# kocurvik/mdrp

Measured on AMD Instinct MI355X. Metric: image-pairs/sec (2000 corrs, 10k RANSAC iters), higher is better.
Workload: dtype f64

## Files before the change

mdrp_amd/csrc/mdrp_capi.hip:

```cpp
#include "../../include/mdrp.h"
#include "mdrp_kernels.h"
#include "mdrp_classic.h"
#include "mdrp_frontend.h"
#ifdef MDRP_SPLIT_TU
#define MDRP_INST extern
#include "mdrp_instances.h"
namespace mdrp {
MDRP_INSTANCES_FINAL_64
MDRP_INSTANCES_FINAL_256
MDRP_INSTANCES_CLASSIC
}
#endif

#include <algorithm>
#include <cmath>
#include <cstdio>
#include <cstdlib>
#include <cstddef>
#include <cstring>
#include <functional>
#include <map>
#include <memory>
#include <mutex>
#include <string>
#include <vector>

using namespace mdrp;

static_assert(sizeof(mdrp_model) == sizeof(Model), "model layout");
static_assert(sizeof(mdrp_camera) == sizeof(CamDev), "camera layout");
static_assert(sizeof(mdrp_result) == sizeof(ResultDev), "result layout");

namespace {

thread_local std::string g_err;

#define HIPCHK(expr)                                                                                       \
    do {                                                                                                   \
        hipError_t e_ = (expr);                                                                            \
        if (e_ != hipSuccess) {                                                                            \
            char buf_[512];                                                                                \
            snprintf(buf_, sizeof buf_, "%s failed: %s (%s:%d)", #expr, hipGetErrorString(e_), __FILE__, __LINE__); \
            g_err = buf_;                                                                                  \
            return MDRP_ERR_HIP;                                                                           \
        }                                                                                                  \
    } while (0)

struct DevBuf {
    void *p = nullptr;
    size_t cap = 0;
    DevBuf() = default;
    DevBuf(const DevBuf &) = delete;
    DevBuf &operator=(const DevBuf &) = delete;
    ~DevBuf() { release(); }
    int ensure(size_t bytes) {
        if (bytes <= cap) return MDRP_OK;
        if (p) { (void)hipFree(p); p = nullptr; cap = 0; }
        size_t want = bytes + bytes / 8 + 256;
        hipError_t e = hipMalloc(&p, want);
        if (e != hipSuccess) { g_err = std::string("hipMalloc failed: ") + hipGetErrorString(e); p = nullptr; return MDRP_ERR_HIP; }
        cap = want;
        return MDRP_OK;
    }
    void release() { if (p) (void)hipFree(p); p = nullptr; cap = 0; }
    template <typename T> T *as() const { return reinterpret_cast<T *>(p); }
};

template <typename T, auto Destroy> struct Owned {
    T v = nullptr;
    Owned() = default;
    Owned(Owned &&o) noexcept : v(o.v) { o.v = nullptr; }
    Owned(const Owned &) = delete;
    Owned &operator=(const Owned &) = delete;
    ~Owned() { reset(); }
    void reset() { if (v) (void)Destroy(v); v = nullptr; }
    operator T() const { return v; }
    T operator->() const { return v; }
};
using Stream = Owned<hipStream_t, hipStreamDestroy>;
using Event = Owned<hipEvent_t, hipEventDestroy>;
template <typename T> using Pinned = Owned<T *, hipHostFree>;

struct Progress {
    int32_t n_active, pad_;
    unsigned long long max_needed;
    unsigned long long evals;
    unsigned long long evals_mfma;
    unsigned long long evals_sweep;
    unsigned long long evals_bound;
    int32_t wish_sum, wish_pairs;
};
struct Counters {
    int32_t unused_[2];
    Progress progress;
    int32_t lo_head[16];
    int32_t xcd_head[8 * LO_XCD_STRIDE];
};
static_assert(offsetof(Counters, progress) == 2 * sizeof(int32_t) && offsetof(Counters, lo_head) == 16 * sizeof(int32_t) &&
              offsetof(Counters, xcd_head) == 32 * sizeof(int32_t) && sizeof(Counters) == 640, "counter block layout");
static_assert(offsetof(Progress, evals_mfma) == offsetof(Progress, evals) + sizeof(unsigned long long), "k_count adds to stats[0] and stats[1]");
static_assert(offsetof(Progress, wish_pairs) == offsetof(Progress, wish_sum) + sizeof(int32_t), "RunParams::inl_stat is [2]");
constexpr size_t LM_STATS_BYTES = 6 * sizeof(unsigned long long);

struct DeviceGuard {
    int prev = -1;
    bool ok = true;
    explicit DeviceGuard(int device) {
        if (hipGetDevice(&prev) != hipSuccess) prev = -1;
        if (prev != device) ok = hipSetDevice(device) == hipSuccess;
    }
    ~DeviceGuard() {
        int cur = -1;
        if (prev >= 0 && hipGetDevice(&cur) == hipSuccess && cur != prev) (void)hipSetDevice(prev);
    }
};

}

struct mdrp_handle {
    std::mutex mu;
    int device = 0;
    hipStream_t stream = nullptr;
    Stream own_stream;
    Stream aux_stream;
    Stream aux_stream2;
    Stream copy_stream;
    Event ev_copied, ev_prepped, ev_solved6;
    DevBuf fuse;
    static constexpr int NC_MAX = 8;
    Event ev_lo, ev_tables, ev_sampled[2], ev_solved[NC_MAX], ev_scanned[NC_MAX];
    int num_cu = 256;
    DevBuf pts, dep, st;
    DevBuf params;
    Pinned<unsigned char> params_host;
    size_t params_host_cap = 0;
    DevBuf models, slot_score, slot_inl, triggers, work_pair, counters, results, mask, plan;
    DevBuf samples[2], tags[2], model_count[2];
    DevBuf tags_sorted[2];
    DevBuf tags_v, surv_count;
    DevBuf cand_stat;
    DevBuf und_count;
    DevBuf rfrag;
    DevBuf cplan;
    DevBuf surv2_count;
    DevBuf lo_mask;
    DevBuf red5;
    DevBuf lm_stats;
    Pinned<unsigned long long> lm_stats_host;
    int64_t fuse_gate_timeouts = 0, fuse_wait_timeouts = 0;
    int64_t first_chunk = 0;
    double seen_wish[3] = {-1.0, -1.0, -1.0};
    Pinned<int32_t> wish_host; Event ev_wish;
    int wish_kind = -1;
    bool fuse_disabled = false;
    int fuse_retry_in = 0;
    int fuse_backoff = 64;
    DevBuf ckpt, ck_list, bresults, bmask;
    int last_budgets = 0;
    DevBuf in_x1, in_x2, in_d1, in_d2;
    DevBuf fe_x1, fe_x2, fe_d1, fe_d2, fe_slot, fe_n;
    Pinned<int32_t> fe_n_host;
    size_t fe_n_host_cap = 0;
    DevBuf unit_a, unit_b, unit_c, unit_d, unit_e, unit_f;
    Pinned<Progress> progress_host;
    std::vector<std::pair<Event, Event>> ev_pool;
    std::vector<int> ev_what;
    size_t ev_used = 0;
    double sweep_ms = 0.0, count_ms = 0.0;
    double kind_ms[6] = {0, 0, 0, 0, 0, 0};
    int64_t kind_launches[6] = {0, 0, 0, 0, 0, 0};
    int64_t lm_cost_evals = 0, lm_accum_evals = 0, fin_cost_evals = 0, fin_accum_evals = 0;
    int64_t count_launches = 0;
    int64_t sweep_launches = 0, sweep_evals = 0, mfma_evals = 0, fp64_evals = 0, bound_evals = 0;
    int last_batch = 0;
};

namespace {

#define MDRP_LM_DISPATCH_T(KERNEL, T, kind, shift, grid, smem, stream, ...)                                          \
    do {                                                                                                             \
        if ((kind) == 0 && (shift)) hipLaunchKernelGGL((KERNEL<0, true, T>), grid, dim3(T), smem, stream, __VA_ARGS__);  \
        else if ((kind) == 0) hipLaunchKernelGGL((KERNEL<0, false, T>), grid, dim3(T), smem, stream, __VA_ARGS__);       \
        else if ((kind) == 1) hipLaunchKernelGGL((KERNEL<1, false, T>), grid, dim3(T), smem, stream, __VA_ARGS__);       \
        else hipLaunchKernelGGL((KERNEL<2, false, T>), grid, dim3(T), smem, stream, __VA_ARGS__);                        \
    } while (0)
#define MDRP_LM_DISPATCH(KERNEL, threads, kind, shift, grid, smem, stream, ...)                                      \
    do {                                                                                                             \
        if ((threads) == 64) MDRP_LM_DISPATCH_T(KERNEL, 64, kind, shift, grid, smem, stream, __VA_ARGS__);           \
        else MDRP_LM_DISPATCH_T(KERNEL, 256, kind, shift, grid, smem, stream, __VA_ARGS__);                          \
    } while (0)

#define MDRP_FINAL_DISPATCH_L(T, FL, kind, shift, grid, smem, stream, ...)                                                  \
    do {                                                                                                                   \
        if ((kind) == 0 && (shift)) hipLaunchKernelGGL((k_final<0, true, T, FL>), grid, dim3(T), smem, stream, __VA_ARGS__);  \
        else if ((kind) == 0) hipLaunchKernelGGL((k_final<0, false, T, FL>), grid, dim3(T), smem, stream, __VA_ARGS__);       \
        else if ((kind) == 1) hipLaunchKernelGGL((k_final<1, false, T, FL>), grid, dim3(T), smem, stream, __VA_ARGS__);       \
        else hipLaunchKernelGGL((k_final<2, false, T, FL>), grid, dim3(T), smem, stream, __VA_ARGS__);                        \
    } while (0)
#define MDRP_FINAL_DISPATCH_T(T, floss, kind, shift, grid, smem, stream, ...)                                               \
    do {                                                                                                                   \
        switch (floss) {                                                                                                   \
        case 1: MDRP_FINAL_DISPATCH_L(T, 1, kind, shift, grid, smem, stream, __VA_ARGS__); break;                          \
        case 2: MDRP_FINAL_DISPATCH_L(T, 2, kind, shift, grid, smem, stream, __VA_ARGS__); break;                          \
        case 3: MDRP_FINAL_DISPATCH_L(T, 3, kind, shift, grid, smem, stream, __VA_ARGS__); break;                          \
        case 4: MDRP_FINAL_DISPATCH_L(T, 4, kind, shift, grid, smem, stream, __VA_ARGS__); break;                          \
        case 5: MDRP_FINAL_DISPATCH_L(T, 5, kind, shift, grid, smem, stream, __VA_ARGS__); break;                          \
        default: MDRP_FINAL_DISPATCH_L(T, 0, kind, shift, grid, smem, stream, __VA_ARGS__); break;  \
        }                                                                                                                  \
    } while (0)
#define MDRP_FINAL_DISPATCH(threads, floss, kind, shift, grid, smem, stream, ...)                                           \
    do {                                                                                                                   \
        if ((threads) == 64) MDRP_FINAL_DISPATCH_T(64, floss, kind, shift, grid, smem, stream, __VA_ARGS__);               \
        else MDRP_FINAL_DISPATCH_T(256, floss, kind, shift, grid, smem, stream, __VA_ARGS__);                              \
    } while (0)

#define MDRP_SWEEP_DISPATCH(KERNEL, kind, grid, block, smem, stream, ...)                                                       \
    do {                                                                                                                        \
        if ((kind) == MDRP_CALIB || (kind) == MDRP_RELPOSE_5PT) hipLaunchKernelGGL((KERNEL<true, false>), grid, block, smem, stream, __VA_ARGS__); \
        else if ((kind) == MDRP_FUNDAMENTAL_7PT) hipLaunchKernelGGL((KERNEL<false, true>), grid, block, smem, stream, __VA_ARGS__); \
        else hipLaunchKernelGGL((KERNEL<false, false>), grid, block, smem, stream, __VA_ARGS__);                                 \
    } while (0)
#define MDRP_CLASSIC_LM_DISPATCH(KERNEL, threads, kind, grid, smem, stream, ...)                                                 \
    do {                                                                                                                        \
        if ((kind) == MDRP_RELPOSE_5PT && (threads) == 64) hipLaunchKernelGGL((KERNEL<CLASSIC_RELPOSE, 64>), grid, dim3(64), smem, stream, __VA_ARGS__); \
        else if ((kind) == MDRP_RELPOSE_5PT) hipLaunchKernelGGL((KERNEL<CLASSIC_RELPOSE, 256>), grid, dim3(256), smem, stream, __VA_ARGS__); \
        else if ((kind) == MDRP_SHARED_6PT && (threads) == 64) hipLaunchKernelGGL((KERNEL<CLASSIC_SHARED, 64>), grid, dim3(64), smem, stream, __VA_ARGS__); \
        else if ((kind) == MDRP_SHARED_6PT) hipLaunchKernelGGL((KERNEL<CLASSIC_SHARED, 256>), grid, dim3(256), smem, stream, __VA_ARGS__); \
        else if ((threads) == 64) hipLaunchKernelGGL((KERNEL<CLASSIC_FUND, 64>), grid, dim3(64), smem, stream, __VA_ARGS__);      \
        else hipLaunchKernelGGL((KERNEL<CLASSIC_FUND, 256>), grid, dim3(256), smem, stream, __VA_ARGS__);                        \
    } while (0)

int env_int(const char *name, int dflt) {
    const char *v = getenv(name);
    return v ? atoi(v) : dflt;
}

int lm_list_stride(int n_max) { return n_max <= LM_LIST_MAX_N ? ((n_max + 63) / 64) * 64 : 0; }
size_t lm_list_bytes(int n_max) { return (size_t)2 * lm_list_stride(n_max) * sizeof(uint16_t); }
int lm_mask_index_on(int n_max) { return lm_list_stride(n_max) > 0 && (size_t)3 * lm_list_stride(n_max) * sizeof(uint16_t) <= 32768 ? 1 : 0; }
size_t lm_final_list_bytes(int n_max) { return (size_t)(2 + lm_mask_index_on(n_max)) * lm_list_stride(n_max) * sizeof(uint16_t); }

int get_events(mdrp_handle *h, hipEvent_t *a, hipEvent_t *b, int what = 0) {
    if (h->ev_used == h->ev_pool.size()) {
        Event x, y;
        HIPCHK(hipEventCreate(&x.v));
        HIPCHK(hipEventCreate(&y.v));
        h->ev_pool.emplace_back(std::move(x), std::move(y));
        h->ev_what.push_back(0);
    }
    h->ev_what[h->ev_used] = what;
    *a = h->ev_pool[h->ev_used].first;
    *b = h->ev_pool[h->ev_used].second;
    h->ev_used++;
    return MDRP_OK;
}

int solver_for(int kind, int est_shift) {
    if (kind == MDRP_CALIB) return est_shift ? SOLVER_SHIFT : SOLVER_P3P;
    return kind == MDRP_SHARED_FOCAL ? SOLVER_SHARED : SOLVER_VARYING;
}

int model_slots(int kind) { return kind == MDRP_RELPOSE_5PT ? 12 : (kind == MDRP_SHARED_6PT ? 16 : 4); }
int sample_size(int kind) { return kind == MDRP_RELPOSE_5PT ? 5 : (kind == MDRP_SHARED_6PT ? 6 : (kind == MDRP_FUNDAMENTAL_7PT ? 7 : 3)); }

bool env_chunks(std::vector<uint64_t> &lead) {
    lead.clear();
    const char *e = getenv("MDRP_CHUNKS");
    if (!e) return false;
    const std::string spec = e;
    size_t pos = 0;
    while (pos < spec.size() && (int)lead.size() < mdrp_handle::NC_MAX - 1) {
        const size_t q = spec.find(',', pos);
        const long v = atol(spec.substr(pos, q == std::string::npos ? std::string::npos : q - pos).c_str());
        if (v > 0) lead.push_back((uint64_t)v);
        if (q == std::string::npos) break;
        pos = q + 1;
    }
    return true;
}

struct PassScratch {
    std::vector<std::pair<DevBuf *, size_t>> bufs;
    size_t fuse;
    size_t params, off_cam1, off_cam2, off_tn, off_tof, off_nper, off_bud;
    size_t red5_blocks, red5_first_blocks;
    size_t total() const {
        size_t t = fuse;
        for (const auto &b : bufs) t += b.second;
        return t;
    }
};

PassScratch pass_scratch(mdrp_handle *h, int kind, int batch, int n_max, int n_tables, int chunk_cap, const std::vector<uint64_t> &lead, int n_budgets = 0) {
    const size_t b = (size_t)batch, n = (size_t)n_max, t = (size_t)n_tables, slots = b * chunk_cap * model_slots(kind);
    PassScratch z;
    z.fuse = 64 + 3 * sizeof(int32_t) * b;
    z.off_cam1 = sizeof(uint64_t) * t; z.off_cam2 = z.off_cam1 + sizeof(CamDev) * b; z.off_tn = z.off_cam2 + sizeof(CamDev) * b;
    z.off_tof = z.off_tn + sizeof(int32_t) * t; z.off_nper = z.off_tof + sizeof(int32_t) * b;
    z.off_bud = (z.off_nper + sizeof(int32_t) * b + 7) / 8 * 8; z.params = n_budgets ? z.off_bud + sizeof(uint64_t) * MAX_BUDGETS : z.off_nper + sizeof(int32_t) * b;
    z.red5_blocks = ((size_t)chunk_cap + 63) / 64;
    z.red5_first_blocks = (std::min<uint64_t>(lead.empty() ? 0 : lead[0], (uint64_t)chunk_cap / 2) + 63) / 64;
    const size_t samples = sizeof(uint32_t) * sample_size(kind) * t * chunk_cap, tags = sizeof(uint32_t) * slots, pair2 = sizeof(int32_t) * 2 * b;
    z.bufs = {
        {&h->pts, sizeof(double) * PT_STRIDE * b * n}, {&h->dep, kind >= MDRP_RELPOSE_5PT ? 0 : sizeof(double) * 2 * b * n}, {&h->st, sizeof(PairState) * b},
        {&h->samples[0], samples}, {&h->params, z.params},
        {&h->models, sizeof(Model) * slots}, {&h->slot_score, sizeof(double) * slots}, {&h->slot_inl, sizeof(int32_t) * slots},
        {&h->tags[0], tags}, {&h->model_count[0], pair2}, {&h->model_count[1], pair2}, {&h->tags[1], tags}, {&h->tags_sorted[0], tags},
        {&h->tags_sorted[1], tags}, {&h->samples[1], samples}, {&h->tags_v, tags},
        {&h->surv_count, sizeof(int32_t) * b}, {&h->cand_stat, sizeof(unsigned long long) * 2 * b}, {&h->und_count, pair2},
        {&h->cplan, sizeof(int32_t) * (b + 1)}, {&h->surv2_count, sizeof(int32_t) * b},
        {&h->rfrag, std::max<size_t>(1024, b * ((n + 15) / 16) * 1024)},
        {&h->triggers, sizeof(Trigger) * b * chunk_cap},
        {&h->work_pair, sizeof(int32_t) * (3 * b + 2)},
        {&h->counters, sizeof(Counters)},
        {&h->plan, sizeof(int32_t) * (2 * b + 2 + 4 + 16)},
        {&h->lo_mask, (kind == MDRP_RELPOSE_5PT || kind == MDRP_SHARED_6PT) ? (size_t)h->num_cu * 8 * std::max<size_t>(n, 1) : 0},
        {&h->red5, kind == MDRP_RELPOSE_5PT ? sizeof(double) * b * (z.red5_blocks + z.red5_first_blocks) * RED5_STRIDE * 64 : 0},
        {&h->ckpt, sizeof(PairState) * b * n_budgets}, {&h->ck_list, sizeof(int32_t) * 3 * b * n_budgets}};
    return z;
}

struct HostSrc { const double *x1, *x2, *d1, *d2; };
struct BudgetOut { const uint64_t *budgets; int n; ResultDev *results; uint8_t *mask; int plane; };

int check_budgets(const mdrp_ransac_opt *ro, const uint64_t *budgets, int n_budgets) {
    const char *why = nullptr;
    if (!ro || !budgets || n_budgets < 1) why = "budgets: an empty list";
    else if (n_budgets > MAX_BUDGETS) why = "budgets: more than MDRP_MAX_BUDGETS";
    else {
        for (int c = 0; c < n_budgets && !why; ++c)
            if (budgets[c] < 1 || (c > 0 && budgets[c] <= budgets[c - 1])) why = "budgets: must be >= 1 and strictly increasing";
        if (!why && budgets[n_budgets - 1] != ro->max_iterations) why = "budgets: ransac_opt.max_iterations must equal the last budget";
    }
    if (why) { g_err = why; return MDRP_ERR_INVALID; }
    return MDRP_OK;
}
constexpr int HOST_SLICE_PAIRS = 256;

int run_pass(mdrp_handle *h, int kind, const double *x1, const double *x2, const double *d1, const double *d2, int batch,
             int n_max, const int32_t *n_host, const mdrp_camera *cam1, const mdrp_camera *cam2, const mdrp_ransac_opt *ro,
             const mdrp_bundle_opt *bo, int chunk_cap, uint8_t *mask_dev, ResultDev *results_dev, const HostSrc *host, int batch_call,
             const BudgetOut *bud = nullptr) {
    hipStream_t s = h->stream;
    const int est_shift = (kind == MDRP_CALIB && ro->monodepth_estimate_shift) ? 1 : 0;
    const bool classic = kind >= MDRP_RELPOSE_5PT;
    const int mps = model_slots(kind), ssz = sample_size(kind);

    std::vector<int32_t> table_of(batch), tab_n;
    {
        std::map<int32_t, int32_t> ids;
        for (int i = 0; i < batch; ++i) {
            auto it = ids.find(n_host[i]);
            if (it == ids.end()) { it = ids.emplace(n_host[i], (int32_t)tab_n.size()).first; tab_n.push_back(n_host[i]); }
            table_of[i] = it->second;
        }
    }
    const int n_tables = (int)tab_n.size();
    std::vector<uint64_t> tab_state(n_tables, ro->seed);

    const uint64_t certain = ro->max_iterations == 0 ? 1 : std::min<uint64_t>(ro->max_iterations, ro->min_iterations + 1);
    std::vector<uint64_t> lead;
    const bool chunks_set = env_chunks(lead);
    if (h->wish_kind >= 0 && hipEventQuery(h->ev_wish) == hipSuccess) {
        if (h->wish_host[1] > 0) h->seen_wish[h->wish_kind] = (double)h->wish_host[0] / (double)h->wish_host[1];
        h->wish_kind = -1;
    }
    if (!chunks_set) {
        if (kind == MDRP_FUNDAMENTAL_7PT) lead = {128, 1024};
        else if (kind == MDRP_SHARED_6PT) lead = {128};
        else if (kind == MDRP_RELPOSE_5PT) lead = {std::min<uint64_t>(512, std::max<uint64_t>(128, certain / 16 / 64 * 64))};
        else {
            lead = {std::min<uint64_t>(256, std::max<uint64_t>(128, certain / 16 / 64 * 64))};
            if (h->seen_wish[kind] >= 0.0 && certain >= 8192)
                lead[0] = (uint64_t)std::min(1024.0, std::max(128.0, std::ceil(h->seen_wish[kind] / 64.0) * 64.0));
        }
    }

    const int n_bud = bud ? bud->n : 0;
    const PassScratch sz = pass_scratch(h, kind, batch, n_max, n_tables, chunk_cap, lead, n_bud);
    int rc;
    for (const auto &b : sz.bufs) {
        if ((rc = b.first->ensure(b.second))) return rc;
        if (b.first == &h->params && h->params_host_cap < sz.params) {
            h->params_host.reset(); h->params_host_cap = 0;
            HIPCHK(hipHostMalloc((void **)&h->params_host.v, sz.params + sz.params / 2, hipHostMallocDefault));
            h->params_host_cap = sz.params + sz.params / 2;
        }
    }
    unsigned char *pd = h->params.as<unsigned char>();
    uint64_t *d_table_state = reinterpret_cast<uint64_t *>(pd);
    CamDev *d_cams1 = reinterpret_cast<CamDev *>(pd + sz.off_cam1), *d_cams2 = reinterpret_cast<CamDev *>(pd + sz.off_cam2);
    int32_t *d_table_n = reinterpret_cast<int32_t *>(pd + sz.off_tn), *d_table_of = reinterpret_cast<int32_t *>(pd + sz.off_tof),
            *d_nper = reinterpret_cast<int32_t *>(pd + sz.off_nper);
    Counters *cnt = h->counters.as<Counters>();
    const size_t groups_max = ((size_t)n_max + 15) / 16;
    const int trig_cap = chunk_cap;

    {
        unsigned char *ph = h->params_host;
        std::memcpy(ph, tab_state.data(), sizeof(uint64_t) * n_tables);
        const bool cams = kind == MDRP_CALIB || kind == MDRP_RELPOSE_5PT || kind == MDRP_SHARED_6PT;
        if (cams) { std::memcpy(ph + sz.off_cam1, cam1, sizeof(CamDev) * batch); std::memcpy(ph + sz.off_cam2, cam2 ? cam2 : cam1, sizeof(CamDev) * batch); }
        else std::memset(ph + sz.off_cam1, 0, 2 * sizeof(CamDev) * (size_t)batch);
        std::memcpy(ph + sz.off_tn, tab_n.data(), sizeof(int32_t) * n_tables);
        std::memcpy(ph + sz.off_tof, table_of.data(), sizeof(int32_t) * batch);
        std::memcpy(ph + sz.off_nper, n_host, sizeof(int32_t) * batch);
        if (bud) std::memcpy(ph + sz.off_bud, bud->budgets, sizeof(uint64_t) * n_bud);
        HIPCHK(hipMemcpyAsync(pd, ph, sz.params, hipMemcpyHostToDevice, s));
    }
    HIPCHK(hipEventRecord(h->ev_tables, s));

    RunParams rp;
    std::memset(&rp, 0, sizeof rp);
    rp.kind = kind; rp.solver = solver_for(kind, est_shift); rp.est_shift = est_shift;
    rp.score_initial = ro->score_initial_model ? 1 : 0;
    rp.batch = batch; rp.n_max = n_max;
    rp.max_iterations = ro->max_iterations; rp.min_iterations = ro->min_iterations;
    rp.dyn_mult = ro->dyn_num_trials_mult; rp.log_prob_missing = std::log(1.0 - ro->success_prob);
    rp.weight_sampson = ro->monodepth_weight_sampson > 0.0f ? (double)ro->monodepth_weight_sampson : 0.0;
    rp.final_max_it = (int)std::min<uint64_t>(bo->max_iterations, 1u << 30); rp.final_loss = bo->loss_type;
    rp.grad_tol = bo->gradient_tol; rp.step_tol = bo->step_tol; rp.lambda0 = bo->initial_lambda;
    rp.lambda_min = bo->min_lambda; rp.lambda_max = bo->max_lambda;
    rp.chunk_len = chunk_cap; rp.chunk_off = 0; rp.slot_stride = chunk_cap * mps; rp.super_len = chunk_cap; rp.chunk_start = 0;
    rp.mps = mps; rp.sample_sz = ssz;

    auto launch_prep = [&](int p0, int pc, hipStream_t ps_) {
        const size_t o2 = (size_t)2 * p0 * n_max, o1 = (size_t)p0 * n_max;
        double *pts_p = h->pts.as<double>() + o1 * PT_STRIDE;
        uint4 *rfrag_p = h->rfrag.as<uint4>() + (size_t)p0 * groups_max * 64;
        if (classic)
            hipLaunchKernelGGL(kc_prep, dim3(pc), dim3(256), 0, ps_, rp, x1 + o2, x2 + o2, d_nper + p0, d_table_of + p0, d_cams1 + p0, d_cams2 + p0,
                               ro->max_epipolar_error, bo->loss_scale, pts_p, h->st.as<PairState>() + p0, rfrag_p);
        else
            hipLaunchKernelGGL(k_prep, dim3(pc), dim3(256), 0, ps_, rp, x1 + o2, x2 + o2, d1 + o1, d2 + o1, d_nper + p0, d_table_of + p0, d_cams1 + p0, d_cams2 + p0,
                               ro->max_epipolar_error, ro->max_reproj_error, bo->loss_scale, pts_p, h->dep.as<double>() + 2 * o1, h->st.as<PairState>() + p0, rfrag_p);
    };
    if (!host) {
        launch_prep(0, batch, s);
        HIPCHK(hipGetLastError());
    }
    rp.inl_stat = classic ? nullptr : &cnt->progress.wish_sum;

    const bool lo_overlap = env_int("MDRP_LO_OVERLAP", 1) != 0;
    const bool use_bound = env_int("MDRP_BOUND", 1) != 0;
    const bool score_split = env_int("MDRP_SCORE_SPLIT", 1) != 0;
    const int lo_threads = env_int("MDRP_LO_THREADS", (batch_call >= 128 && n_max < 4096) ? 64 : 256);
    const int final_threads = env_int("MDRP_FINAL_THREADS", batch_call >= 4096 ? 64 : 256);
    const int mask_index = lm_mask_index_on(n_max);
    const int clm_list_stride = lm_list_stride(n_max);
    const size_t clm_list_bytes = (size_t)2 * clm_list_stride * sizeof(uint16_t);
    const bool fuse_env = !bud && env_int("MDRP_FUSE_TAIL", ((kind == MDRP_CALIB && est_shift) || h->fuse_disabled) ? 0 : 1) != 0;
    bool final_done = false;
    auto launch_final_of = [&](const RunParams &rf, int problems, PairState *st_f, uint8_t *mask_f, ResultDev *results_f, const int32_t *ready, int32_t *fin_done,
                               unsigned long long ticks, unsigned long long *timeouts) {
        if (classic)
            MDRP_CLASSIC_LM_DISPATCH(kc_final, final_threads, kind, dim3(problems), clm_list_bytes, s, rf, st_f, h->pts.as<double>(), mask_f, results_f,
                                     ready, fin_done, ticks, timeouts, clm_list_stride);
        else
            MDRP_FINAL_DISPATCH(final_threads, rf.final_loss, kind, est_shift, dim3(problems), (mask_index ? lm_final_list_bytes(n_max) : lm_list_bytes(n_max)), s, rf,
                                st_f, h->pts.as<double>(), h->dep.as<double>(), mask_f, results_f, lm_list_stride(n_max), mask_index,
                                h->lm_stats.as<unsigned long long>() + 2, ready, fin_done, ticks, timeouts);
    };
    auto launch_final = [&](const int32_t *ready, int32_t *fin_done, unsigned long long ticks, unsigned long long *timeouts) {
        launch_final_of(rp, batch, h->st.as<PairState>(), mask_dev, results_dev, ready, fin_done, ticks, timeouts);
    };
    const size_t tile_bytes = SCORE_TILE_BYTES;

    uint64_t it0 = 0;
    uint64_t max_needed = 0;
    while (true) {
        uint64_t lens[mdrp_handle::NC_MAX] = {0};
        int n_chunks = 1;
        if (it0 < certain) {
            const uint64_t span = std::min<uint64_t>(certain - it0, (uint64_t)chunk_cap);
            uint64_t used = 0;
            n_chunks = 0;
            if (it0 == 0)
                for (uint64_t l : lead) {
                    if (used + 2 * l > span) break;
                    lens[n_chunks++] = l; used += l;
                }
            lens[n_chunks++] = span - used;
        } else {
            lens[0] = std::min<uint64_t>(std::min<uint64_t>(std::max<uint64_t>(max_needed, 256), ro->max_iterations - it0), (uint64_t)chunk_cap);
        }
        uint64_t super_len = 0;
        for (int c = 0; c < n_chunks; ++c) super_len += lens[c];
        if (it0 == 0) h->first_chunk = (int64_t)lens[0];
        rp.chunk_start = it0; rp.super_len = (int)super_len;
        HIPCHK(hipMemsetAsync(h->counters.p, 0, sizeof(Counters), s));
        if (it0 == 0) HIPCHK(hipMemsetAsync(h->cand_stat.p, 0, sizeof(unsigned long long) * 2 * batch, s));
        const bool piped = n_chunks > 1 && lo_overlap;
        const bool fuse_tail = fuse_env && piped && it0 + super_len >= ro->max_iterations;
        int32_t *fz_ctl = nullptr, *fz_done = nullptr, *fz_fin = nullptr, *fz_ready = nullptr;
        if (fuse_tail) {
            if ((rc = h->fuse.ensure(sz.fuse))) return rc;
            fz_ctl = h->fuse.as<int32_t>(); fz_done = fz_ctl + 16; fz_fin = fz_done + batch; fz_ready = fz_fin + batch;
        }
        hipStream_t aux = piped ? h->aux_stream : s, aux2 = piped ? h->aux_stream2 : s;
        int offs[mdrp_handle::NC_MAX] = {0};
        for (int c = 1; c < n_chunks; ++c) offs[c] = offs[c - 1] + (int)lens[c - 1];
        const int samp_threads = env_int("MDRP_SAMPLE_THREADS", ssz == 3 ? SAMP_THREADS : (ssz == 5 ? 512 : 256));
        auto launch_samples = [&](hipStream_t st_, int len_, uint32_t *smp_) {
            if (ssz == 6) hipLaunchKernelGGL(kc_samples<6>, dim3(n_tables), dim3(samp_threads), 0, st_, n_tables, d_table_n, d_table_state, len_, smp_);
            else if (ssz == 5) hipLaunchKernelGGL(kc_samples<5>, dim3(n_tables), dim3(samp_threads), 0, st_, n_tables, d_table_n, d_table_state, len_, smp_);
            else if (ssz == 7) hipLaunchKernelGGL(kc_samples<7>, dim3(n_tables), dim3(samp_threads), 0, st_, n_tables, d_table_n, d_table_state, len_, smp_);
            else hipLaunchKernelGGL(k_samples, dim3(n_tables), dim3(samp_threads), 0, st_, n_tables, d_table_n, d_table_state, len_, smp_);
        };
        bool presampled[2] = {false, false};
        if (piped && it0 == 0) {
            HIPCHK(hipStreamWaitEvent(aux2, h->ev_tables, 0));
            for (int c = 0; c < 2 && c < n_chunks; ++c) {
                launch_samples(aux2, (int)lens[c], h->samples[c & 1].as<uint32_t>());
                HIPCHK(hipEventRecord(h->ev_sampled[c], aux2));
                presampled[c] = true;
            }
        }
        auto issue_solve = [&](int c, hipStream_t st_, int p0, int pc) -> int {
            RunParams r = rp;
            r.chunk_len = (int)lens[c]; r.chunk_off = offs[c]; r.batch = pc;
            const size_t so = (size_t)p0 * rp.slot_stride;
            uint32_t *tg = h->tags[c & 1].as<uint32_t>() + so;
            uint32_t *smp = h->samples[c & 1].as<uint32_t>();
            int32_t *mc = h->model_count[c & 1].as<int32_t>() + 2 * (size_t)p0;
            HIPCHK(hipMemsetAsync(mc, 0, sizeof(int32_t) * 2 * pc, st_));
            if (c < 2 && presampled[c]) HIPCHK(hipStreamWaitEvent(st_, h->ev_sampled[c], 0));
            else launch_samples(st_, r.chunk_len, smp);
            hipEvent_t v0, v1;
            int rc_;
            if ((rc_ = get_events(h, &v0, &v1, 5))) return rc_;
            HIPCHK(hipEventRecord(v0, st_));
            struct Stop { hipEvent_t e; hipStream_t s; ~Stop() { (void)hipEventRecord(e, s); } } stop_{v1, st_};
            PairState *st_p = h->st.as<PairState>() + p0;
            double *pts_p = h->pts.as<double>() + (size_t)p0 * n_max * PT_STRIDE;
            Model *models_p = h->models.as<Model>() + so;
            int32_t *inl_p = h->slot_inl.as<int32_t>() + so;
            if (classic) {
                const dim3 sgrid((r.chunk_len + 63) / 64, pc);
                if (kind == MDRP_SHARED_6PT)
                    hipLaunchKernelGGL(kc_solve<CLASSIC_SHARED>, sgrid, dim3(64), 0, st_, r, st_p, smp, pts_p, models_p, inl_p, tg, mc);
                else if (kind == MDRP_RELPOSE_5PT) {
                    const bool first_region = c == 0 && n_chunks > 1;
                    if (first_region && (size_t)sgrid.x > sz.red5_first_blocks) { g_err = "5-point first chunk longer than its Reduce5 region"; return MDRP_ERR_INVALID; }
                    double *red5 = h->red5.as<double>() + ((first_region ? (size_t)batch * sz.red5_blocks : 0) + (size_t)p0 * sgrid.x) * RED5_STRIDE * 64;
                    hipLaunchKernelGGL(kc_solve5_null, sgrid, dim3(64), SOLVE5N_LDS_BYTES, st_, r, st_p, smp, pts_p, red5);
                    hipLaunchKernelGGL(kc_solve5_reduce, sgrid, dim3(64), SOLVE5_LDS_BYTES, st_, r, st_p, red5);
                    hipLaunchKernelGGL(kc_solve5_roots, sgrid, dim3(64), SOLVE5B_LDS_BYTES, st_, r, st_p, smp, pts_p, red5, models_p, inl_p, tg, mc);
                }
                else
                    hipLaunchKernelGGL(kc_solve<CLASSIC_FUND>, sgrid, dim3(64), SOLVE7_LDS_BYTES, st_, r, st_p, smp, pts_p, models_p, inl_p, tg, mc);
                return MDRP_OK;
            }
            double *dep_p = h->dep.as<double>() + (size_t)p0 * n_max * 2;
#define MDRP_SOLVE_LAUNCH(S)                                                                                                   \
    hipLaunchKernelGGL(k_solve<S>, dim3((r.chunk_len + solve_threads(S) - 1) / solve_threads(S), pc), dim3(solve_threads(S)), 0, st_, r, st_p, smp, pts_p, dep_p, models_p, inl_p, tg, mc, 0, r.chunk_len)
            switch (r.solver) {
            case SOLVER_P3P: MDRP_SOLVE_LAUNCH(SOLVER_P3P); break;
            case SOLVER_SHIFT: MDRP_SOLVE_LAUNCH(SOLVER_SHIFT); break;
            case SOLVER_SHARED: MDRP_SOLVE_LAUNCH(SOLVER_SHARED); break;
            default: MDRP_SOLVE_LAUNCH(SOLVER_VARYING); break;
            }
#undef MDRP_SOLVE_LAUNCH
            return MDRP_OK;
        };
        auto sweep_chunk = [&](int c, int p0, int pc) -> int {
            RunParams r = rp;
            r.chunk_len = (int)lens[c]; r.chunk_off = offs[c]; r.batch = pc;
            const int len = r.chunk_len;
            const bool odd = c & 1;
            const size_t so = (size_t)p0 * rp.slot_stride;
            PairState *st_p = h->st.as<PairState>() + p0;
            const double *pts_p = h->pts.as<double>() + (size_t)p0 * n_max * PT_STRIDE;
            const Model *models_p = h->models.as<Model>() + so;
            uint32_t *tags_sc = h->tags_sorted[odd].as<uint32_t>() + so;
            int32_t *mcount_c = h->model_count[odd].as<int32_t>() + 2 * (size_t)p0;
            uint32_t *tags_c = h->tags[odd].as<uint32_t>() + so;
            uint32_t *tags_v = h->tags_v.as<uint32_t>() + so;
            int32_t *surv1 = h->surv_count.as<int32_t>() + p0, *surv2 = h->surv2_count.as<int32_t>() + p0;
            hipEvent_t e0, e1;
            int rc_;
            if ((rc_ = get_events(h, &e0, &e1, 0))) return rc_;
            unsigned long long *cstats = &cnt->progress.evals;
            {
                hipEvent_t c0, c1;
                if ((rc_ = get_events(h, &c0, &c1, 1))) return rc_;
                const bool two_phase = !(it0 == 0 && c == 0);
                unsigned long long *cand_stat = h->cand_stat.as<unsigned long long>() + 2 * (size_t)p0;
                uint32_t *tags_u = tags_sc;
                int32_t *und_part = reinterpret_cast<int32_t *>(h->tags_sorted[!odd].as<uint32_t>() + so), *und_cnt = h->und_count.as<int32_t>() + 2 * (size_t)p0;
                const uint4 *rfrag_p = h->rfrag.as<uint4>() + (size_t)p0 * groups_max * 64;
                hipLaunchKernelGGL(k_count_plan, dim3(1), dim3(PLAN_THREADS), 0, s, pc, st_p, mcount_c, 2, CNT_WG_MODELS, h->cplan.as<int32_t>(),
                                   surv1, (const int32_t *)nullptr, two_phase ? und_cnt : (int32_t *)nullptr);
                const dim3 cgrid((unsigned)pc * (unsigned)((len * mps + CNT_WG_MODELS - 1) / CNT_WG_MODELS));
                HIPCHK(hipEventRecord(c0, s));
                MDRP_SWEEP_DISPATCH(k_count, kind, cgrid, dim3(CNT_THREADS), 0, s, r, st_p, rfrag_p, models_p,
                                    tags_c, mcount_c, h->cplan.as<int32_t>(), tags_v, surv1, cstats, (int32_t *)nullptr, (const int32_t *)nullptr,
                                    1, tags_u, und_part, und_cnt, (const int32_t *)nullptr, cand_stat);
                if (two_phase) {
                    hipLaunchKernelGGL(k_count_plan, dim3(1), dim3(PLAN_THREADS), 0, s, pc, st_p, und_cnt, 2, CNT_WG_MODELS, h->cplan.as<int32_t>(),
                                       (int32_t *)nullptr, (const int32_t *)nullptr, (int32_t *)nullptr);
                    MDRP_SWEEP_DISPATCH(k_count, kind, cgrid, dim3(CNT_THREADS), 0, s, r, st_p, rfrag_p, models_p,
                                        tags_u, und_cnt, h->cplan.as<int32_t>(), tags_v, surv1, cstats, (int32_t *)nullptr, (const int32_t *)nullptr,
                                        2, (uint32_t *)nullptr, (int32_t *)nullptr, (int32_t *)nullptr, und_part, cand_stat);
                    h->count_launches++;
                }
                HIPCHK(hipEventRecord(c1, s));
                h->count_launches++;
            }
            const uint32_t *surv_tags = tags_v;
            const int32_t *surv_cnt = surv1;
            if (use_bound && batch_call > 16 && !(it0 == 0 && c == 0)) {
                hipLaunchKernelGGL(k_count_plan, dim3(1), dim3(PLAN_THREADS), 0, s, pc, st_p, surv1, 1, BND_THREADS, h->cplan.as<int32_t>(), surv2, (const int32_t *)nullptr);
                const dim3 bgrid((unsigned)pc * (unsigned)((len * mps + BND_THREADS - 1) / BND_THREADS));
                unsigned long long *bstats = &cnt->progress.evals_bound;
                hipEvent_t b0, b1;
                if ((rc_ = get_events(h, &b0, &b1, 4))) return rc_;
                HIPCHK(hipEventRecord(b0, s));
                MDRP_SWEEP_DISPATCH(k_bound, kind, bgrid, dim3(BND_THREADS), 0, s, r, st_p, pts_p, models_p, tags_v, surv1, h->cplan.as<int32_t>(), tags_c, surv2, bstats);
                HIPCHK(hipEventRecord(b1, s));
                surv_tags = tags_c; surv_cnt = surv2;
            }
            int32_t *plan = h->plan.as<int32_t>(), *totals = plan + 2 * (size_t)batch + 2;
            if (batch_call <= SCORE_WAVE_MAX_PAIRS) {
                hipLaunchKernelGGL(k_count_plan, dim3(1), dim3(PLAN_THREADS), 0, s, pc, st_p, surv_cnt, 1, SCW_THREADS / 64, plan, (int32_t *)nullptr, (const int32_t *)nullptr, (int32_t *)nullptr);
                hipLaunchKernelGGL(k_sort_tags, dim3(pc), dim3(256), 0, s, r, st_p, mcount_c, surv_cnt, surv_tags, tags_sc);
                HIPCHK(hipEventRecord(e0, s));
                const long long ub = (long long)pc * ((len * mps + SCW_THREADS / 64 - 1) / (SCW_THREADS / 64));
                const dim3 grid((unsigned)std::min<long long>(ub, (long long)h->num_cu * 32));
                MDRP_SWEEP_DISPATCH(k_score_w, kind, grid, dim3(SCW_THREADS), 0, s, r, st_p, pts_p, models_p, tags_sc, mcount_c,
                                    h->slot_score.as<double>() + so, h->slot_inl.as<int32_t>() + so, plan);
            } else if (score_split && !(it0 == 0 && c == 0)) {
                hipLaunchKernelGGL(k_sort_tags, dim3(pc), dim3(256), 0, s, r, st_p, mcount_c, surv_cnt, surv_tags, tags_sc);
                hipLaunchKernelGGL(k_plan, dim3(1), dim3(PLAN_THREADS), 0, s, pc, mcount_c, plan, totals, SPLIT_HYP);
                HIPCHK(hipEventRecord(e0, s));
                const long long ub = (long long)pc * ((len * mps + SPLIT_HYP - 1) / SPLIT_HYP + 1);
                const dim3 grid((unsigned)std::min<long long>(ub, (long long)h->num_cu * 32));
                MDRP_SWEEP_DISPATCH(k_score_split, kind, grid, dim3(SPLIT_THREADS), 0, s, r, st_p, pts_p, models_p, tags_sc, mcount_c,
                                    h->slot_score.as<double>() + so, h->slot_inl.as<int32_t>() + so, plan, totals);
            } else {
                hipLaunchKernelGGL(k_sort_tags, dim3(pc), dim3(256), 0, s, r, st_p, mcount_c, surv_cnt, surv_tags, tags_sc);
                hipLaunchKernelGGL(k_plan, dim3(1), dim3(PLAN_THREADS), 0, s, pc, mcount_c, plan, totals, SCORE_THREADS);
                HIPCHK(hipEventRecord(e0, s));
                const dim3 grid((unsigned)pc * (unsigned)((len * mps + SCORE_THREADS - 1) / SCORE_THREADS));
                MDRP_SWEEP_DISPATCH(k_score, kind, grid, dim3(SCORE_THREADS), tile_bytes, s, r, st_p, pts_p, models_p, tags_sc, mcount_c,
                                    h->slot_score.as<double>() + so, h->slot_inl.as<int32_t>() + so, plan, totals);
            }
            HIPCHK(hipEventRecord(e1, s));
            h->sweep_launches++;
            Trigger *trig_p = h->triggers.as<Trigger>() + (size_t)p0 * trig_cap;
            unsigned long long *scan_stats = &cnt->progress.evals_sweep;
#define MDRP_SCAN(M, I) hipLaunchKernelGGL((k_scan<M, I>), dim3(pc), dim3(64), 0, s, r, st_p, h->slot_score.as<double>() + so, h->slot_inl.as<int32_t>() + so, trig_p, trig_cap, mcount_c, scan_stats)
            if (mps == 16) MDRP_SCAN(16, 1);
            else if (mps == 12) MDRP_SCAN(12, 1);
            else if (len >= 1024) MDRP_SCAN(4, 4);
            else MDRP_SCAN(4, 1);
#undef MDRP_SCAN
            return MDRP_OK;
        };
        bool solved1 = false;
        int swept0 = 0;
        if (host && it0 == 0) {
            const bool sliced = piped && n_chunks >= 2 && batch >= 2 * HOST_SLICE_PAIRS;
            const int sl = sliced ? HOST_SLICE_PAIRS : batch;
            for (int p0 = 0; p0 < batch; p0 += sl) {
                const int pc = std::min(sl, batch - p0);
                const size_t o2 = (size_t)2 * p0 * n_max, o1 = (size_t)p0 * n_max, n2 = sizeof(double) * 2 * (size_t)pc * n_max, n1 = sizeof(double) * (size_t)pc * n_max;
                hipStream_t cs = sliced ? h->copy_stream : s;
                HIPCHK(hipMemcpyAsync(const_cast<double *>(x1) + o2, host->x1 + o2, n2, hipMemcpyHostToDevice, cs));
                HIPCHK(hipMemcpyAsync(const_cast<double *>(x2) + o2, host->x2 + o2, n2, hipMemcpyHostToDevice, cs));
                if (host->d1 && host->d2) {
                    HIPCHK(hipMemcpyAsync(const_cast<double *>(d1) + o1, host->d1 + o1, n1, hipMemcpyHostToDevice, cs));
                    HIPCHK(hipMemcpyAsync(const_cast<double *>(d2) + o1, host->d2 + o1, n1, hipMemcpyHostToDevice, cs));
                }
                if (!sliced) { launch_prep(p0, pc, s); break; }
                HIPCHK(hipEventRecord(h->ev_copied, cs)); HIPCHK(hipStreamWaitEvent(aux, h->ev_copied, 0));
                if (p0 == 0) HIPCHK(hipStreamWaitEvent(aux, h->ev_tables, 0));
                launch_prep(p0, pc, aux);
                HIPCHK(hipEventRecord(h->ev_prepped, aux));
                if ((rc = issue_solve(1, aux, p0, pc))) return rc;
                const bool last = p0 + sl >= batch, last_but_one = !last && p0 + 2 * sl >= batch;
                if (last_but_one || last) HIPCHK(hipStreamWaitEvent(s, h->ev_prepped, 0));
                auto solve_first = [&](int q0, int qc) -> int {
                    if (kind != MDRP_SHARED_6PT) return issue_solve(0, s, q0, qc);
                    int rc_ = issue_solve(0, aux, q0, qc);
                    if (rc_) return rc_;
                    HIPCHK(hipEventRecord(h->ev_solved6, aux));
                    HIPCHK(hipStreamWaitEvent(s, h->ev_solved6, 0));
                    return MDRP_OK;
                };
                if (last_but_one) { swept0 = p0 + pc; if ((rc = solve_first(0, swept0)) || (rc = sweep_chunk(0, 0, swept0))) return rc; }
                if (last) { if ((rc = solve_first(swept0, batch - swept0)) || (rc = sweep_chunk(0, swept0, batch - swept0))) return rc; swept0 = batch; }
            }
            if (sliced) { HIPCHK(hipEventRecord(h->ev_solved[1], aux)); solved1 = true; }
        }
        if (swept0 < batch && (rc = issue_solve(0, s, 0, batch))) return rc;
        if (piped) HIPCHK(hipEventRecord(h->ev_solved[0], s));
        for (int c = 0; c < n_chunks; ++c) {
            rp.chunk_len = (int)lens[c]; rp.chunk_off = offs[c];
            if (c == 0 && swept0 >= batch) {
                if (piped) HIPCHK(hipEventRecord(h->ev_scanned[0], s));
                continue;
            }
            if (piped && c + 1 < n_chunks && !(c == 0 && solved1)) {
                HIPCHK(hipStreamWaitEvent(aux, c == 0 ? h->ev_solved[0] : h->ev_scanned[c - 1], 0));
                if ((rc = issue_solve(c + 1, aux, 0, batch))) return rc;
                HIPCHK(hipEventRecord(h->ev_solved[c + 1], aux));
            }
            if (piped && c > 0) HIPCHK(hipStreamWaitEvent(s, h->ev_solved[c], 0));
            if (!piped && c > 0 && (rc = issue_solve(c, s, 0, batch))) return rc;
            if ((rc = sweep_chunk(c, 0, batch))) return rc;
            if (c + 1 < n_chunks) {
                if (piped) HIPCHK(hipEventRecord(h->ev_scanned[c], s));
                continue;
            }
            int32_t *lo_plan = h->work_pair.as<int32_t>();
            hipLaunchKernelGGL(k_lo_plan, dim3(1), dim3(PLAN_THREADS), 0, s, batch, h->st.as<PairState>(), (const int32_t *)nullptr, lo_plan);
            if (fuse_tail) {
                HIPCHK(hipMemsetAsync(fz_ctl, 0, 64 + 2 * sizeof(int32_t) * (size_t)batch, s));
                HIPCHK(hipMemsetAsync(fz_ready, 0xFF, sizeof(int32_t) * (size_t)batch, s));
            }
            if (piped) { HIPCHK(hipEventRecord(h->ev_scanned[c], s)); HIPCHK(hipStreamWaitEvent(aux2, h->ev_scanned[c], 0)); }
            const int lo_blocks = h->num_cu * (lo_threads == 64 ? 8 : 2);
            const FuseTail fz = fuse_tail ? FuseTail{fz_done, fz_ready, fz_ctl, h->st.as<PairState>()} : FuseTail{nullptr, nullptr, nullptr, nullptr};
            unsigned long long *lm_stats = h->lm_stats.as<unsigned long long>();
            int32_t *xheads = cnt->xcd_head;
            hipEvent_t l0, l1;
            if ((rc = get_events(h, &l0, &l1, 2))) return rc;
            HIPCHK(hipEventRecord(l0, aux2));
            if (classic)
                MDRP_CLASSIC_LM_DISPATCH(kc_lo, lo_threads, kind, dim3(lo_blocks), clm_list_bytes, aux2, rp, h->st.as<PairState>(), h->pts.as<double>(),
                                         h->models.as<Model>(), h->triggers.as<Trigger>(), trig_cap, lo_plan, cnt->lo_head, xheads,
                                         h->lo_mask.as<uint8_t>(), clm_list_stride, fz);
            else
                MDRP_LM_DISPATCH(k_lo, lo_threads, kind, est_shift, dim3(lo_blocks), lm_list_bytes(n_max), aux2, rp,
                                 h->st.as<PairState>(), h->pts.as<double>(), h->dep.as<double>(), h->models.as<Model>(), h->triggers.as<Trigger>(),
                                 trig_cap, lo_plan, cnt->lo_head, xheads, lm_list_stride(n_max), lm_stats, fz);
            HIPCHK(hipEventRecord(l1, aux2));
        }
        if (fuse_tail) {
            const int32_t *plan_l = h->work_pair.as<int32_t>();
            const int lo_blocks_l = h->num_cu * (lo_threads == 64 ? 8 : 2);
            const long long n_scale = std::max(1, (n_max + 1999) / 2000);
            const unsigned long long gate_ticks = 100ull * (unsigned long long)env_int("MDRP_FUSE_GATE_US", (int)std::min<long long>((50000 + 40ll * batch) * n_scale, 200000));
            const unsigned long long wait_ticks = 100ull * (unsigned long long)env_int("MDRP_FUSE_WAIT_US", (int)std::min<long long>((20000 + 4ll * batch) * n_scale, 100000));
            hipLaunchKernelGGL(k_gate, dim3(1), dim3(1), 0, s, (const int32_t *)cnt->lo_head, plan_l + 3 * (size_t)batch + 1,
                               (const int32_t *)fz_ctl, lo_blocks_l, gate_ticks, h->lm_stats.as<unsigned long long>() + 4);
            hipEvent_t g0, g1;
            if ((rc = get_events(h, &g0, &g1, 3))) return rc;
            HIPCHK(hipEventRecord(g0, s));
            launch_final(fz_ready, fz_fin, wait_ticks, h->lm_stats.as<unsigned long long>() + 5);
            HIPCHK(hipEventRecord(g1, s));
            final_done = true;
        }
        if (piped) { HIPCHK(hipEventRecord(h->ev_lo, aux2)); HIPCHK(hipStreamWaitEvent(s, h->ev_lo, 0)); }
        if (fuse_tail)
            launch_final(nullptr, fz_fin, 0, nullptr);
        if (bud)
            hipLaunchKernelGGL(k_walk_ckpt, dim3((batch + WALK_CKPT_THREADS - 1) / WALK_CKPT_THREADS), dim3(WALK_CKPT_THREADS), 0, s, rp, h->st.as<PairState>(), h->models.as<Model>(),
                               h->triggers.as<Trigger>(), trig_cap, &cnt->progress.n_active, &cnt->progress.max_needed,
                               reinterpret_cast<const uint64_t *>(pd + sz.off_bud), n_bud, h->ckpt.as<PairState>());
        else if (!fuse_tail)
            hipLaunchKernelGGL(k_walk, dim3((batch + 63) / 64), dim3(64), 0, s, rp, h->st.as<PairState>(), h->models.as<Model>(),
                               h->triggers.as<Trigger>(), trig_cap, &cnt->progress.n_active, &cnt->progress.max_needed,
                               (const int32_t *)nullptr, 0, 0, 0);
        HIPCHK(hipGetLastError());
        HIPCHK(hipMemcpyAsync(h->progress_host, &cnt->progress, sizeof(Progress), hipMemcpyDeviceToHost, s));
        HIPCHK(hipStreamSynchronize(s));
        h->sweep_evals += (int64_t)h->progress_host->evals;
        h->mfma_evals += (int64_t)h->progress_host->evals_mfma;
        h->fp64_evals += (int64_t)h->progress_host->evals_sweep;
        h->bound_evals += (int64_t)h->progress_host->evals_bound;
        if (final_done && h->progress_host->wish_pairs > 0)
            h->seen_wish[kind] = (double)h->progress_host->wish_sum / (double)h->progress_host->wish_pairs;
        if (getenv("MDRP_DEBUG"))
            fprintf(stderr, "[mdrp] super-chunk start %llu len %llu (%d chunks): evals %llu (mfma %llu, fp32 bound %llu, fp64 sweep %llu = %.2f %%) active %d max_needed %llu\n",
                    (unsigned long long)it0, (unsigned long long)super_len, n_chunks, h->progress_host->evals, h->progress_host->evals_mfma,
                    h->progress_host->evals_bound, h->progress_host->evals_sweep, 100.0 * (double)h->progress_host->evals_sweep / (double)std::max<unsigned long long>(1, h->progress_host->evals),
                    h->progress_host->n_active, h->progress_host->max_needed);
        it0 += super_len;
        if (h->progress_host->n_active == 0 || it0 >= ro->max_iterations) break;
        max_needed = h->progress_host->max_needed;
    }

    if (final_done) return MDRP_OK;
    hipEvent_t f0, f1;
    if ((rc = get_events(h, &f0, &f1, 3))) return rc;
    HIPCHK(hipEventRecord(f0, s));
    if (bud) {
        const int problems = n_bud * batch;
        int32_t *list = h->ck_list.as<int32_t>(), *rep = list + problems, *done = rep + problems;
        hipLaunchKernelGGL(k_ckpt_plan, dim3(1), dim3(PLAN_THREADS), 0, s, batch, n_bud, h->ckpt.as<PairState>(), list, rep);
        RunParams rf = rp;
        rf.ck_pairs = batch; rf.ck_plane = bud->plane;
        rf.inl_stat = nullptr;
        launch_final_of(rf, problems, h->ckpt.as<PairState>(), bud->mask, bud->results, list, done, 0, nullptr);
        rf.inl_stat = rp.inl_stat;
        hipLaunchKernelGGL(k_ckpt_fill, dim3(problems), dim3(CKPT_FILL_THREADS), 0, s, rf, n_bud, h->ckpt.as<PairState>(), rep, bud->results, bud->mask);
    } else
        launch_final(nullptr, nullptr, 0, nullptr);
    HIPCHK(hipEventRecord(f1, s));
    if (rp.inl_stat && h->wish_kind < 0) {
        HIPCHK(hipMemcpyAsync(h->wish_host, rp.inl_stat, 2 * sizeof(int32_t), hipMemcpyDeviceToHost, s));
        HIPCHK(hipEventRecord(h->ev_wish, s));
        h->wish_kind = kind;
    }
    HIPCHK(hipGetLastError());
    return MDRP_OK;
}

int estimate_device(mdrp_handle *h, int kind, const double *x1, const double *x2, const double *d1, const double *d2, int batch,
                    int n_max, const int32_t *n_per_pair, const mdrp_camera *cam1, const mdrp_camera *cam2,
                    const mdrp_ransac_opt *ro, const mdrp_bundle_opt *bo, uint8_t *mask_dev, const HostSrc *host = nullptr,
                    const uint64_t *budgets = nullptr, int n_budgets = 0) {
    const bool known_kind = kind >= 0 && kind <= 5;
    if (!h || batch < 0 || n_max < 0 || !known_kind || !ro || !bo) { g_err = "invalid argument"; return MDRP_ERR_INVALID; }
    if (kind == MDRP_SHARED_6PT && batch > 0 && !cam1) { g_err = "the 6-point estimator needs the principal point in cam1"; return MDRP_ERR_INVALID; }
    if ((kind == MDRP_CALIB || kind == MDRP_RELPOSE_5PT) && batch > 0 && (!cam1 || !cam2)) { g_err = "calibrated estimator needs cameras"; return MDRP_ERR_INVALID; }
    if (kind <= 2 && batch > 0 && n_max > 0 && (!d1 || !d2)) { g_err = "monodepth estimator needs depths"; return MDRP_ERR_INVALID; }
    if (ro->progressive_sampling) { g_err = "progressive_sampling (PROSAC, RandomSampler::initialize_prosac) is not built"; return MDRP_ERR_UNSUPPORTED; }
    if (ro->real_focal_check && (kind == MDRP_SHARED_6PT || kind == MDRP_FUNDAMENTAL_7PT)) { g_err = "real_focal_check is not built"; return MDRP_ERR_UNSUPPORTED; }
    h->last_budgets = n_budgets;
    if (h->fuse_disabled && --h->fuse_retry_in <= 0) h->fuse_disabled = false;
    h->ev_used = 0; h->sweep_ms = 0; h->sweep_launches = 0; h->sweep_evals = 0; h->mfma_evals = 0; h->fp64_evals = 0; h->bound_evals = 0; h->count_launches = 0; h->count_ms = 0; h->last_batch = batch; h->lm_cost_evals = 0; h->lm_accum_evals = 0;
    int rc;
    if ((rc = h->results.ensure(sizeof(ResultDev) * std::max(batch, 1)))) return rc;
    if ((rc = h->lm_stats.ensure(LM_STATS_BYTES))) return rc;
    HIPCHK(hipMemsetAsync(h->lm_stats.p, 0, LM_STATS_BYTES, h->stream));
    if (batch == 0) return MDRP_OK;
    std::vector<int32_t> n_host(batch);
    for (int i = 0; i < batch; ++i) {
        n_host[i] = n_per_pair ? n_per_pair[i] : n_max;
        if (n_host[i] < 0 || n_host[i] > n_max) { g_err = "n_per_pair out of range"; return MDRP_ERR_INVALID; }
    }
    uint8_t *mask = mask_dev;
    if (!mask) {
        if ((rc = (budgets ? h->bmask : h->mask).ensure((size_t)std::max(n_budgets, 1) * batch * std::max(n_max, 1)))) return rc;
        mask = (budgets ? h->bmask : h->mask).as<uint8_t>();
    }
    if (budgets && (rc = h->bresults.ensure(sizeof(ResultDev) * n_budgets * batch))) return rc;
    uint64_t chunk_cap64 = std::min<uint64_t>(std::max<uint64_t>(ro->max_iterations, 1), std::max<uint64_t>(ro->min_iterations + 1, 4096));
    chunk_cap64 = std::min<uint64_t>(chunk_cap64, 16384);
    const int chunk_cap = (int)chunk_cap64;
    size_t free_b = 0, total_b = 0;
    HIPCHK(hipMemGetInfo(&free_b, &total_b));
    std::vector<uint64_t> lead;
    if (!env_chunks(lead)) lead.assign(1, 512);
    const size_t per_pair = pass_scratch(h, kind, 2, n_max, 2, chunk_cap, lead, n_budgets).total() - pass_scratch(h, kind, 1, n_max, 1, chunk_cap, lead, n_budgets).total();
    size_t budget = std::min<size_t>((size_t)(0.5 * (double)free_b), (size_t)96 << 30);
    int per_pass = (int)std::max<size_t>(1, std::min<size_t>((size_t)batch, budget / per_pair));
    per_pass = std::min(per_pass, 65535);
    per_pass = std::max(1, std::min(per_pass, env_int("MDRP_PAIRS_PER_PASS", per_pass)));
    for (int p0 = 0; p0 < batch; p0 += per_pass) {
        const int nb = std::min(per_pass, batch - p0);
        HostSrc hs{};
        if (host) hs = HostSrc{host->x1 + (size_t)2 * p0 * n_max, host->x2 + (size_t)2 * p0 * n_max, host->d1 ? host->d1 + (size_t)p0 * n_max : nullptr,
                               host->d2 ? host->d2 + (size_t)p0 * n_max : nullptr};
        const BudgetOut bud{budgets, n_budgets, h->bresults.as<ResultDev>() + p0, mask + (size_t)p0 * n_max, batch};
        rc = run_pass(h, kind, x1 + (size_t)2 * p0 * n_max, x2 + (size_t)2 * p0 * n_max, d1 ? d1 + (size_t)p0 * n_max : nullptr,
                      d2 ? d2 + (size_t)p0 * n_max : nullptr, nb,
                      n_max, n_host.data() + p0, cam1 ? cam1 + p0 : nullptr, cam2 ? cam2 + p0 : nullptr, ro, bo, chunk_cap,
                      mask + (size_t)p0 * n_max, h->results.as<ResultDev>() + p0, host ? &hs : nullptr, batch, budgets ? &bud : nullptr);
        if (rc) return rc;
    }
    if (budgets) {
        HIPCHK(hipMemcpyAsync(h->results.p, h->bresults.as<ResultDev>() + (size_t)(n_budgets - 1) * batch, sizeof(ResultDev) * batch, hipMemcpyDeviceToDevice, h->stream));
    }
    return MDRP_OK;
}

int finish_timing(mdrp_handle *h) {
    if (h->lm_stats.p) HIPCHK(hipMemcpyAsync(h->lm_stats_host, h->lm_stats.p, LM_STATS_BYTES, hipMemcpyDeviceToHost, h->stream));
    HIPCHK(hipStreamSynchronize(h->stream));
    h->lm_cost_evals = (int64_t)h->lm_stats_host[0]; h->lm_accum_evals = (int64_t)h->lm_stats_host[1];
    h->fin_cost_evals = (int64_t)h->lm_stats_host[2]; h->fin_accum_evals = (int64_t)h->lm_stats_host[3];
    h->fuse_gate_timeouts = (int64_t)h->lm_stats_host[4]; h->fuse_wait_timeouts = (int64_t)h->lm_stats_host[5];
    if (!(h->fuse_gate_timeouts || h->fuse_wait_timeouts) && !h->fuse_disabled) h->fuse_backoff = 64;
    if ((h->fuse_gate_timeouts || h->fuse_wait_timeouts) && !h->fuse_disabled) {
        h->fuse_disabled = true;
        h->fuse_retry_in = h->fuse_backoff;
        h->fuse_backoff = std::min(h->fuse_backoff * 2, 16384);
        if (!getenv("MDRP_QUIET"))
            fprintf(stderr, "[mdrp] fused tail: %lld gate / %lld final-refinement waits timed out (kernels of two streams did not overlap: "
                            "profiler or serialised dispatch?); this handle runs unfused for its next %d calls\n",
                    (long long)h->fuse_gate_timeouts, (long long)h->fuse_wait_timeouts, h->fuse_retry_in);
    }
    for (int k = 0; k < 6; ++k) { h->kind_ms[k] = 0; h->kind_launches[k] = 0; }
    for (size_t i = 0; i < h->ev_used; ++i) {
        float t = 0;
        HIPCHK(hipEventElapsedTime(&t, h->ev_pool[i].first, h->ev_pool[i].second));
        const int k = std::min(std::max(h->ev_what[i], 0), 5);
        h->kind_ms[k] += t; h->kind_launches[k]++;
    }
    h->sweep_ms = h->kind_ms[0]; h->count_ms = h->kind_ms[1];
    return MDRP_OK;
}

}

#define MDRP_ENTER(h)                                                                      \
    std::lock_guard<std::mutex> lock_((h)->mu);                                            \
    DeviceGuard guard_((h)->device);                                                       \
    if (!guard_.ok) { g_err = "hipSetDevice failed"; return MDRP_ERR_HIP; }

#ifndef MDRP_SRC_HASH
#define MDRP_SRC_HASH "unknown"
#endif

static int create_handle(int device, hipStream_t stream, bool own_stream, mdrp_handle **out);

extern "C" {

const char *mdrp_last_error(void) { return g_err.c_str(); }
int mdrp_abi_version(void) { return MDRP_ABI_VERSION; }
const char *mdrp_version(void) { return "mdrp-hip 0.6 (gfx950) MDRP_SRC_HASH=" MDRP_SRC_HASH; }

int mdrp_hip_build_version(void) { return HIP_VERSION; }

static int check_host_abi(int abi_version, int ransac_opt_bytes) {
    if (abi_version == MDRP_ABI_VERSION && ransac_opt_bytes == (int)sizeof(mdrp_ransac_opt)) return MDRP_OK;
    char buf[256];
    snprintf(buf, sizeof buf, "host was compiled against ABI %#x (mdrp_ransac_opt %d bytes), this library speaks %#x (%d bytes): recompile the host against include/mdrp.h",
             abi_version, ransac_opt_bytes, MDRP_ABI_VERSION, (int)sizeof(mdrp_ransac_opt));
    g_err = buf;
    return MDRP_ERR_INVALID;
}
int mdrp_create_(int device, void *stream, mdrp_handle **out, int abi_version, int ransac_opt_bytes) {
    if (int rc = check_host_abi(abi_version, ransac_opt_bytes)) return rc;
    return create_handle(device, (hipStream_t)stream, stream == nullptr, out);
}
int mdrp_create_on_stream_(int device, void *stream, mdrp_handle **out, int abi_version, int ransac_opt_bytes) {
    if (int rc = check_host_abi(abi_version, ransac_opt_bytes)) return rc;
    return create_handle(device, (hipStream_t)stream, false, out);
}

}

static int create_handle(int device, hipStream_t stream, bool own_stream, mdrp_handle **out) {
    if (!out) return MDRP_ERR_INVALID;
    int ndev = 0;
    if (hipGetDeviceCount(&ndev) != hipSuccess || ndev <= 0 || device < 0 || device >= ndev) {
        g_err = "no usable HIP device";
        return MDRP_ERR_NO_DEVICE;
    }
    DeviceGuard guard_(device);
    if (!guard_.ok) { g_err = "hipSetDevice failed"; return MDRP_ERR_HIP; }
    std::unique_ptr<mdrp_handle> h(new mdrp_handle());
    h->device = device;
    if (own_stream) HIPCHK(hipStreamCreateWithFlags(&h->own_stream.v, hipStreamNonBlocking));
    h->stream = own_stream ? h->own_stream.v : stream;
    hipDeviceProp_t prop;
    HIPCHK(hipGetDeviceProperties(&prop, device));
    h->num_cu = prop.multiProcessorCount > 0 ? prop.multiProcessorCount : 256;
    HIPCHK(hipHostMalloc((void **)&h->progress_host.v, sizeof(Progress), hipHostMallocDefault));
    HIPCHK(hipHostMalloc((void **)&h->lm_stats_host.v, LM_STATS_BYTES, hipHostMallocDefault));
    HIPCHK(hipHostMalloc((void **)&h->wish_host.v, 2 * sizeof(int32_t), hipHostMallocDefault));
    HIPCHK(hipEventCreateWithFlags(&h->ev_wish.v, hipEventDisableTiming));
    std::memset(h->lm_stats_host, 0, LM_STATS_BYTES);
    {
        int prio_lo = 0, prio_hi = 0;
        (void)hipDeviceGetStreamPriorityRange(&prio_lo, &prio_hi);
        HIPCHK(hipStreamCreateWithPriority(&h->aux_stream.v, hipStreamNonBlocking, prio_hi));
        HIPCHK(hipStreamCreateWithPriority(&h->aux_stream2.v, hipStreamNonBlocking, prio_hi));
    }
    HIPCHK(hipStreamCreateWithFlags(&h->copy_stream.v, hipStreamNonBlocking));
    for (Event *e : {&h->ev_copied, &h->ev_prepped, &h->ev_solved6, &h->ev_lo, &h->ev_tables, &h->ev_sampled[0], &h->ev_sampled[1]})
        HIPCHK(hipEventCreateWithFlags(&e->v, hipEventDisableTiming));
    for (int i = 0; i < mdrp_handle::NC_MAX; ++i) {
        HIPCHK(hipEventCreateWithFlags(&h->ev_solved[i].v, hipEventDisableTiming));
        HIPCHK(hipEventCreateWithFlags(&h->ev_scanned[i].v, hipEventDisableTiming));
    }
    const int tile_bytes = (int)SCORE_TILE_BYTES;
    HIPCHK(hipFuncSetAttribute(reinterpret_cast<const void *>(k_score<true>), hipFuncAttributeMaxDynamicSharedMemorySize, tile_bytes));
    HIPCHK(hipFuncSetAttribute(reinterpret_cast<const void *>(k_score<false>), hipFuncAttributeMaxDynamicSharedMemorySize, tile_bytes));
    HIPCHK(hipFuncSetAttribute(reinterpret_cast<const void *>(k_score<false, true>), hipFuncAttributeMaxDynamicSharedMemorySize, tile_bytes));
    HIPCHK(hipFuncSetAttribute(reinterpret_cast<const void *>(kc_solve5_reduce), hipFuncAttributeMaxDynamicSharedMemorySize, (int)SOLVE5_LDS_BYTES));
    HIPCHK(hipFuncSetAttribute(reinterpret_cast<const void *>(kc_solver_unit<CLASSIC_RELPOSE>), hipFuncAttributeMaxDynamicSharedMemorySize, (int)SOLVE5_LDS_BYTES));
    *out = h.release();
    return MDRP_OK;
}

static int upload_iota(hipStream_t s, void *tags, int count) {
    std::vector<uint32_t> iota(count);
    for (int i = 0; i < count; ++i) iota[i] = (uint32_t)i;
    HIPCHK(hipMemcpyAsync(tags, iota.data(), sizeof(uint32_t) * count, hipMemcpyHostToDevice, s));
    return MDRP_OK;
}
static int stage_unit_pair(mdrp_handle *h, const double *x1, const double *x2, int n, double sq_threshold) {
    hipStream_t s = h->stream;
    PairState ps;
    std::memset(&ps, 0, sizeof ps);
    ps.n = n; ps.active = 1; ps.sq_thr = sq_threshold; ps.eps = std::sqrt(sq_threshold);
    ps.best_min_score = DBL_MAX;
    HIPCHK(hipMemcpyAsync(h->st.p, &ps, sizeof ps, hipMemcpyHostToDevice, s));
    hipLaunchKernelGGL(k_pack_unit, dim3((n + 255) / 256 + 1), dim3(256), 0, s, n, x1, x2, (const double *)nullptr,
                       (const double *)nullptr, h->pts.as<double>(), (double *)nullptr);
    hipLaunchKernelGGL(k_box_unit, dim3(1), dim3(256), 0, s, n, h->pts.as<double>(), h->st.as<PairState>());
    return MDRP_OK;
}

static LmOpt lm_opt(const mdrp_bundle_opt *opt) {
    LmOpt o;
    o.max_it = (int)std::min<uint64_t>(opt->max_iterations, 1u << 30); o.loss = opt->loss_type; o.loss_scale = opt->loss_scale;
    o.grad_tol = opt->gradient_tol; o.step_tol = opt->step_tol; o.lambda0 = opt->initial_lambda;
    o.lambda_min = opt->min_lambda; o.lambda_max = opt->max_lambda;
    return o;
}

extern "C" {

void mdrp_destroy(mdrp_handle *h) {
    if (!h) return;
    DeviceGuard guard_(h->device);
    for (hipStream_t st : {h->stream, (hipStream_t)h->aux_stream, (hipStream_t)h->aux_stream2, (hipStream_t)h->copy_stream}) (void)hipStreamSynchronize(st);
    delete h;
}

int mdrp_synchronize(mdrp_handle *h) {
    if (!h) return MDRP_ERR_INVALID;
    MDRP_ENTER(h);
    HIPCHK(hipStreamSynchronize(h->stream));
    return MDRP_OK;
}

int mdrp_estimate_batch_async(mdrp_handle *h, int kind, const double *x1, const double *x2, const double *d1, const double *d2,
                              int batch, int n_max, const int32_t *n_per_pair, const mdrp_camera *cam1, const mdrp_camera *cam2,
                              const mdrp_ransac_opt *ropt, const mdrp_bundle_opt *bopt, uint8_t *inlier_mask_dev) {
    if (!h) { g_err = "invalid argument"; return MDRP_ERR_INVALID; }
    MDRP_ENTER(h);
    return estimate_device(h, kind, x1, x2, d1, d2, batch, n_max, n_per_pair, cam1, cam2, ropt, bopt, inlier_mask_dev);
}

static int fetch_results_locked(mdrp_handle *h, mdrp_result *out, int batch) {
    if (!out || batch < 0 || batch > h->last_batch) { g_err = "invalid argument"; return MDRP_ERR_INVALID; }
    HIPCHK(hipMemcpyAsync(out, h->results.p, sizeof(ResultDev) * batch, hipMemcpyDeviceToHost, h->stream));
    return finish_timing(h);
}

int mdrp_copy_results_device(mdrp_handle *h, void *dst_dev, int batch) {
    if (!h || !dst_dev || batch < 0 || batch > h->last_batch) { g_err = "invalid argument"; return MDRP_ERR_INVALID; }
    MDRP_ENTER(h);
    HIPCHK(hipMemcpyAsync(dst_dev, h->results.p, sizeof(ResultDev) * batch, hipMemcpyDeviceToDevice, h->stream));
    return finish_timing(h);
}

int mdrp_fetch_results(mdrp_handle *h, mdrp_result *out, int batch) {
    if (!h) { g_err = "invalid argument"; return MDRP_ERR_INVALID; }
    MDRP_ENTER(h);
    return fetch_results_locked(h, out, batch);
}

int mdrp_estimate_batch(mdrp_handle *h, int kind, int mem_space, const double *x1, const double *x2, const double *d1,
                        const double *d2, int batch, int n_max, const int32_t *n_per_pair, const mdrp_camera *cam1,
                        const mdrp_camera *cam2, const mdrp_ransac_opt *ropt, const mdrp_bundle_opt *bopt, mdrp_result *out,
                        uint8_t *inlier_mask) {
    if (!h || !out || batch < 0 || n_max < 0) { g_err = "invalid argument"; return MDRP_ERR_INVALID; }
    MDRP_ENTER(h);
    const size_t np = (size_t)batch * n_max;
    int rc;
    uint8_t *mask_dev = inlier_mask;
    HostSrc hsrc{};
    bool use_host = false;
    if (mem_space == MDRP_MEM_HOST) {
        if ((rc = h->in_x1.ensure(sizeof(double) * 2 * np + 16)) || (rc = h->in_x2.ensure(sizeof(double) * 2 * np + 16)) ||
            (rc = h->in_d1.ensure(sizeof(double) * np + 16)) || (rc = h->in_d2.ensure(sizeof(double) * np + 16)))
            return rc;
        hsrc = HostSrc{x1, x2, (d1 && d2) ? d1 : nullptr, (d1 && d2) ? d2 : nullptr};
        if (d1 && d2) { d1 = h->in_d1.as<double>(); d2 = h->in_d2.as<double>(); }
        x1 = h->in_x1.as<double>(); x2 = h->in_x2.as<double>();
        use_host = true;
        mask_dev = nullptr;
    }
    rc = estimate_device(h, kind, x1, x2, d1, d2, batch, n_max, n_per_pair, cam1, cam2, ropt, bopt, mask_dev, use_host ? &hsrc : nullptr);
    if (rc) return rc;
    if (mem_space == MDRP_MEM_HOST && inlier_mask && np > 0)
        HIPCHK(hipMemcpyAsync(inlier_mask, h->mask.p, np, hipMemcpyDeviceToHost, h->stream));
    return fetch_results_locked(h, out, batch);
}

static_assert(MDRP_MAX_BUDGETS == MAX_BUDGETS, "budget limit of the header and of the kernels");

static int drain_and_return(mdrp_handle *h, int rc) {
    for (hipStream_t st : {h->stream, (hipStream_t)h->aux_stream, (hipStream_t)h->aux_stream2, (hipStream_t)h->copy_stream}) (void)hipStreamSynchronize(st);
    return rc;
}

static int budget_results_locked(mdrp_handle *h, void *dst, int n_budgets, int batch, hipMemcpyKind where) {
    if (!dst || batch < 0 || n_budgets < 1 || n_budgets != h->last_budgets || batch != h->last_batch) {
        g_err = "budget results: n_budgets and batch must be those of the handle's last budgets call";
        return MDRP_ERR_INVALID;
    }
    if (batch > 0) HIPCHK(hipMemcpyAsync(dst, h->bresults.p, sizeof(ResultDev) * n_budgets * batch, where, h->stream));
    return finish_timing(h);
}

int mdrp_estimate_batch_budgets_async(mdrp_handle *h, int kind, const double *x1, const double *x2, const double *d1, const double *d2,
                                      int batch, int n_max, const int32_t *n_per_pair, const mdrp_camera *cam1, const mdrp_camera *cam2,
                                      const mdrp_ransac_opt *ropt, const mdrp_bundle_opt *bopt, const uint64_t *budgets, int n_budgets,
                                      uint8_t *inlier_mask_dev) {
    if (!h) { g_err = "invalid argument"; return MDRP_ERR_INVALID; }
    if (int rc = check_budgets(ropt, budgets, n_budgets)) return rc;
    MDRP_ENTER(h);
    const int rc = estimate_device(h, kind, x1, x2, d1, d2, batch, n_max, n_per_pair, cam1, cam2, ropt, bopt, inlier_mask_dev, nullptr, budgets, n_budgets);
    return rc ? drain_and_return(h, rc) : rc;
}

int mdrp_fetch_budget_results(mdrp_handle *h, mdrp_result *out, int n_budgets, int batch) {
    if (!h) { g_err = "invalid argument"; return MDRP_ERR_INVALID; }
    MDRP_ENTER(h);
    return budget_results_locked(h, out, n_budgets, batch, hipMemcpyDeviceToHost);
}

int mdrp_copy_budget_results_device(mdrp_handle *h, void *dst_dev, int n_budgets, int batch) {
    if (!h) { g_err = "invalid argument"; return MDRP_ERR_INVALID; }
    MDRP_ENTER(h);
    return budget_results_locked(h, dst_dev, n_budgets, batch, hipMemcpyDeviceToDevice);
}

int mdrp_estimate_batch_budgets(mdrp_handle *h, int kind, int mem_space, const double *x1, const double *x2, const double *d1,
                                const double *d2, int batch, int n_max, const int32_t *n_per_pair, const mdrp_camera *cam1,
                                const mdrp_camera *cam2, const mdrp_ransac_opt *ropt, const mdrp_bundle_opt *bopt, const uint64_t *budgets,
                                int n_budgets, mdrp_result *out, uint8_t *inlier_mask) {
    if (!h || !out || batch < 0 || n_max < 0) { g_err = "invalid argument"; return MDRP_ERR_INVALID; }
    if (int rc = check_budgets(ropt, budgets, n_budgets)) return rc;
    MDRP_ENTER(h);
    const size_t np = (size_t)batch * n_max;
    int rc;
    uint8_t *mask_dev = inlier_mask;
    HostSrc hsrc{};
    bool use_host = false;
    if (mem_space == MDRP_MEM_HOST) {
        if ((rc = h->in_x1.ensure(sizeof(double) * 2 * np + 16)) || (rc = h->in_x2.ensure(sizeof(double) * 2 * np + 16)) ||
            (rc = h->in_d1.ensure(sizeof(double) * np + 16)) || (rc = h->in_d2.ensure(sizeof(double) * np + 16)))
            return rc;
        hsrc = HostSrc{x1, x2, (d1 && d2) ? d1 : nullptr, (d1 && d2) ? d2 : nullptr};
        if (d1 && d2) { d1 = h->in_d1.as<double>(); d2 = h->in_d2.as<double>(); }
        x1 = h->in_x1.as<double>(); x2 = h->in_x2.as<double>();
        use_host = true;
        mask_dev = nullptr;
    }
    rc = estimate_device(h, kind, x1, x2, d1, d2, batch, n_max, n_per_pair, cam1, cam2, ropt, bopt, mask_dev, use_host ? &hsrc : nullptr, budgets, n_budgets);
    if (rc) return drain_and_return(h, rc);
    if (mem_space == MDRP_MEM_HOST && inlier_mask && np > 0 &&
        hipMemcpyAsync(inlier_mask, h->bmask.p, np * n_budgets, hipMemcpyDeviceToHost, h->stream) != hipSuccess) {
        g_err = "copy of the inlier masks failed";
        return drain_and_return(h, MDRP_ERR_HIP);
    }
    rc = budget_results_locked(h, out, n_budgets, batch, hipMemcpyDeviceToHost);
    return rc ? drain_and_return(h, rc) : rc;
}

}

static int check_matches(const mdrp_matches *mm, int batch) {
    const char *why = nullptr;
    if (!mm || batch < 0) why = "invalid argument";
    else if ((mm->kp_type != MDRP_F32 && mm->kp_type != MDRP_F64) || (mm->depth_type != MDRP_F32 && mm->depth_type != MDRP_F64)) why = "kp_type / depth_type must be MDRP_F32 or MDRP_F64";
    else if (mm->filter != MDRP_FILTER_BOTH_INF && mm->filter != MDRP_FILTER_FINITE) why = "unknown filter";
    else if (mm->k1 < 0 || mm->k2 < 0 || mm->m_max < 0 || mm->h1 < 0 || mm->w1 < 0 || mm->h2 < 0 || mm->w2 < 0) why = "negative size";
    else if (batch > 0 && mm->m_max > 0 &&
             (!mm->matches || (mm->k1 > 0 && !mm->kp1) || (mm->k2 > 0 && !mm->kp2) || (mm->h1 > 0 && mm->w1 > 0 && !mm->depth1) ||
              (mm->h2 > 0 && mm->w2 > 0 && !mm->depth2)))
        why = "NULL keypoints, matches or depth map";
    if (why) { g_err = std::string("mdrp_matches: ") + why; return MDRP_ERR_INVALID; }
    return MDRP_OK;
}

static int gather_device(mdrp_handle *h, const mdrp_matches *mm, int batch, double *x1, double *x2, double *d1, double *d2, int32_t *slot, int32_t *n_dev) {
    if (batch == 0) return MDRP_OK;
#define MDRP_GATHER(KT, DT)                                                                                                                \
    hipLaunchKernelGGL((k_gather<KT, DT>), dim3(batch), dim3(FE_THREADS), 0, h->stream, (const KT *)mm->kp1, (const KT *)mm->kp2, mm->k1, mm->k2,  \
                       mm->matches, mm->m_max, (const DT *)mm->depth1, (const DT *)mm->depth2, mm->h1, mm->w1, mm->h2, mm->w2, mm->center1,      \
                       mm->center2, mm->filter, x1, x2, d1, d2, slot, n_dev)
    if (mm->kp_type == MDRP_F32 && mm->depth_type == MDRP_F32) MDRP_GATHER(float, float);
    else if (mm->kp_type == MDRP_F32) MDRP_GATHER(float, double);
    else if (mm->depth_type == MDRP_F32) MDRP_GATHER(double, float);
    else MDRP_GATHER(double, double);
#undef MDRP_GATHER
    HIPCHK(hipGetLastError());
    return MDRP_OK;
}

static int fetch_counts(mdrp_handle *h, int batch) {
    if (batch == 0) return MDRP_OK;
    if ((size_t)batch > h->fe_n_host_cap) {
        h->fe_n_host.reset();
        h->fe_n_host_cap = 0;
        HIPCHK(hipHostMalloc((void **)&h->fe_n_host.v, sizeof(int32_t) * ((size_t)batch + batch / 8 + 64), hipHostMallocDefault));
        h->fe_n_host_cap = (size_t)batch + batch / 8 + 64;
    }
    HIPCHK(hipMemcpyAsync(h->fe_n_host, h->fe_n.p, sizeof(int32_t) * batch, hipMemcpyDeviceToHost, h->stream));
    HIPCHK(hipStreamSynchronize(h->stream));
    return MDRP_OK;
}

extern "C" {

int mdrp_gather_matches(mdrp_handle *h, const mdrp_matches *mm, int batch, double *x1, double *x2, double *d1, double *d2, int32_t *slot,
                        int32_t *n_host) {
    if (!h) { g_err = "invalid argument"; return MDRP_ERR_INVALID; }
    if (int rc = check_matches(mm, batch)) return rc;
    if (batch > 0 && (!n_host || (mm->m_max > 0 && (!x1 || !x2 || !d1 || !d2 || !slot)))) { g_err = "mdrp_gather_matches: NULL output"; return MDRP_ERR_INVALID; }
    MDRP_ENTER(h);
    int rc;
    if ((rc = h->fe_n.ensure(sizeof(int32_t) * std::max(batch, 1)))) return rc;
    if ((rc = gather_device(h, mm, batch, x1, x2, d1, d2, slot, h->fe_n.as<int32_t>()))) return rc;
    if ((rc = fetch_counts(h, batch))) return rc;
    if (batch > 0) std::memcpy(n_host, h->fe_n_host, sizeof(int32_t) * batch);
    return MDRP_OK;
}

int mdrp_estimate_matches_async(mdrp_handle *h, int kind, const mdrp_matches *mm, int batch, const mdrp_camera *cam1, const mdrp_camera *cam2,
                                const mdrp_ransac_opt *ropt, const mdrp_bundle_opt *bopt, uint8_t *match_mask_dev, int32_t *n_used_host) {
    if (!h || !ropt || !bopt) { g_err = "invalid argument"; return MDRP_ERR_INVALID; }
    if (kind != MDRP_CALIB && kind != MDRP_SHARED_FOCAL && kind != MDRP_VARYING_FOCAL) {
        g_err = "mdrp_estimate_matches_async: only the monodepth estimators (kind 0..2) take depth maps";
        return MDRP_ERR_INVALID;
    }
    if (int rc = check_matches(mm, batch)) return rc;
    MDRP_ENTER(h);
    const size_t rows = (size_t)batch * mm->m_max;
    int rc;
    if ((rc = h->fe_x1.ensure(sizeof(double) * 2 * rows + 16)) || (rc = h->fe_x2.ensure(sizeof(double) * 2 * rows + 16)) ||
        (rc = h->fe_d1.ensure(sizeof(double) * rows + 16)) || (rc = h->fe_d2.ensure(sizeof(double) * rows + 16)) ||
        (rc = h->fe_slot.ensure(sizeof(int32_t) * rows + 16)) || (rc = h->fe_n.ensure(sizeof(int32_t) * std::max(batch, 1))))
        return rc;
    if ((rc = gather_device(h, mm, batch, h->fe_x1.as<double>(), h->fe_x2.as<double>(), h->fe_d1.as<double>(), h->fe_d2.as<double>(),
                            h->fe_slot.as<int32_t>(), h->fe_n.as<int32_t>())))
        return rc;
    if ((rc = fetch_counts(h, batch))) return rc;
    rc = estimate_device(h, kind, h->fe_x1.as<double>(), h->fe_x2.as<double>(), h->fe_d1.as<double>(), h->fe_d2.as<double>(), batch, mm->m_max,
                         batch > 0 ? h->fe_n_host.v : nullptr, cam1, cam2, ropt, bopt, nullptr);
    if (rc) return rc;
    if (match_mask_dev && rows > 0) {
        hipLaunchKernelGGL(k_match_mask, dim3((unsigned)((rows + FE_THREADS - 1) / FE_THREADS)), dim3(FE_THREADS), 0, h->stream, h->fe_slot.as<int32_t>(),
                           h->mask.as<uint8_t>(), mm->m_max, rows, match_mask_dev);
        HIPCHK(hipGetLastError());
    }
    if (n_used_host && batch > 0) std::memcpy(n_used_host, h->fe_n_host, sizeof(int32_t) * batch);
    return MDRP_OK;
}

}

extern "C" {

int mdrp_last_sweep_stats(mdrp_handle *h, double *sweep_ms, int64_t *launches, int64_t *evaluations) {
    if (!h) return MDRP_ERR_INVALID;
    std::lock_guard<std::mutex> lock_(h->mu);
    if (sweep_ms) *sweep_ms = h->sweep_ms;
    if (launches) *launches = h->sweep_launches;
    if (evaluations) *evaluations = h->sweep_evals;
    return MDRP_OK;
}

int mdrp_last_stats_sized(mdrp_handle *h, mdrp_stats *out, size_t out_size) {
    if (!h || !out || out_size < sizeof(double)) return MDRP_ERR_INVALID;
    std::lock_guard<std::mutex> lock_(h->mu);
    mdrp_stats full, *caller = out;
    out = &full;
    out->count_ms = h->count_ms; out->count_launches = h->count_launches;
    out->sweep_ms = h->sweep_ms; out->sweep_launches = h->sweep_launches;
    out->evals_algorithmic = h->sweep_evals; out->evals_mfma = h->mfma_evals; out->evals_fp64 = h->fp64_evals; out->evals_bound = h->bound_evals;
    out->lo_ms = h->kind_ms[2]; out->lo_launches = h->kind_launches[2]; out->final_ms = h->kind_ms[3]; out->final_launches = h->kind_launches[3];
    out->bound_ms = h->kind_ms[4]; out->bound_launches = h->kind_launches[4]; out->solve_ms = h->kind_ms[5]; out->solve_launches = h->kind_launches[5];
    out->lm_cost_evals = h->lm_cost_evals; out->lm_accum_evals = h->lm_accum_evals;
    out->final_cost_evals = h->fin_cost_evals; out->final_accum_evals = h->fin_accum_evals;
    out->fuse_gate_timeouts = h->fuse_gate_timeouts; out->fuse_wait_timeouts = h->fuse_wait_timeouts;
    out->first_chunk = h->first_chunk;
    std::memcpy(caller, &full, std::min(out_size, sizeof full));
    return MDRP_OK;
}

int mdrp_last_stats(mdrp_handle *h, mdrp_stats *out) { return mdrp_last_stats_sized(h, out, offsetof(mdrp_stats, fuse_gate_timeouts)); }

int mdrp_solver_batch(mdrp_handle *h, int solver, const double *x1h, const double *x2h, const double *d1, const double *d2,
                      int count, mdrp_model *out, int32_t *n_out) {
    if (!h || count < 0 || solver < 0 || solver > 3 || !out || !n_out) { g_err = "invalid argument"; return MDRP_ERR_INVALID; }
    if (count == 0) return MDRP_OK;
    MDRP_ENTER(h);
    int rc;
    if ((rc = h->unit_a.ensure(sizeof(double) * 9 * count)) || (rc = h->unit_b.ensure(sizeof(double) * 9 * count)) ||
        (rc = h->unit_c.ensure(sizeof(double) * 3 * count)) || (rc = h->unit_d.ensure(sizeof(double) * 3 * count)) ||
        (rc = h->unit_e.ensure(sizeof(Model) * 4 * count)) || (rc = h->unit_f.ensure(sizeof(int32_t) * count)))
        return rc;
    hipStream_t s = h->stream;
    HIPCHK(hipMemcpyAsync(h->unit_a.p, x1h, sizeof(double) * 9 * count, hipMemcpyHostToDevice, s));
    HIPCHK(hipMemcpyAsync(h->unit_b.p, x2h, sizeof(double) * 9 * count, hipMemcpyHostToDevice, s));
    HIPCHK(hipMemcpyAsync(h->unit_c.p, d1, sizeof(double) * 3 * count, hipMemcpyHostToDevice, s));
    HIPCHK(hipMemcpyAsync(h->unit_d.p, d2, sizeof(double) * 3 * count, hipMemcpyHostToDevice, s));
    HIPCHK(hipMemsetAsync(h->unit_e.p, 0, sizeof(Model) * 4 * count, s));
    hipLaunchKernelGGL(k_solver_unit, dim3((count + 63) / 64), dim3(64), 0, s, solver, count, h->unit_a.as<double>(),
                       h->unit_b.as<double>(), h->unit_c.as<double>(), h->unit_d.as<double>(), h->unit_e.as<Model>(), h->unit_f.as<int32_t>());
    HIPCHK(hipGetLastError());
    HIPCHK(hipMemcpyAsync(out, h->unit_e.p, sizeof(Model) * 4 * count, hipMemcpyDeviceToHost, s));
    HIPCHK(hipMemcpyAsync(n_out, h->unit_f.p, sizeof(int32_t) * count, hipMemcpyDeviceToHost, s));
    HIPCHK(hipStreamSynchronize(s));
    return MDRP_OK;
}

int mdrp_classic_solver_batch(mdrp_handle *h, int kind, const double *x1h, const double *x2h, int count, mdrp_model *out, int32_t *n_out) {
    if (!h || count < 0 || kind < MDRP_RELPOSE_5PT || kind > MDRP_FUNDAMENTAL_7PT || !out || !n_out) { g_err = "invalid argument"; return MDRP_ERR_INVALID; }
    if (count == 0) return MDRP_OK;
    MDRP_ENTER(h);
    const int K = kind == MDRP_RELPOSE_5PT ? 5 : (kind == MDRP_SHARED_6PT ? 6 : 7), M = kind == MDRP_RELPOSE_5PT ? MAX_MODELS_5PT : (kind == MDRP_SHARED_6PT ? MAX_MODELS_6PT : 3);
    int rc;
    if ((rc = h->unit_a.ensure(sizeof(double) * 3 * K * count)) || (rc = h->unit_b.ensure(sizeof(double) * 3 * K * count)) ||
        (rc = h->unit_e.ensure(sizeof(Model) * M * count)) || (rc = h->unit_f.ensure(sizeof(int32_t) * count)))
        return rc;
    hipStream_t s = h->stream;
    HIPCHK(hipMemcpyAsync(h->unit_a.p, x1h, sizeof(double) * 3 * K * count, hipMemcpyHostToDevice, s));
    HIPCHK(hipMemcpyAsync(h->unit_b.p, x2h, sizeof(double) * 3 * K * count, hipMemcpyHostToDevice, s));
    HIPCHK(hipMemsetAsync(h->unit_e.p, 0, sizeof(Model) * M * count, s));
    if (kind == MDRP_SHARED_6PT)
        hipLaunchKernelGGL(kc_solver_unit<CLASSIC_SHARED>, dim3((count + 63) / 64), dim3(64), 0, s, count, h->unit_a.as<double>(),
                           h->unit_b.as<double>(), h->unit_e.as<Model>(), h->unit_f.as<int32_t>());
    else if (kind == MDRP_RELPOSE_5PT)
        hipLaunchKernelGGL(kc_solver_unit<CLASSIC_RELPOSE>, dim3((count + 63) / 64), dim3(64), SOLVE5_LDS_BYTES, s, count, h->unit_a.as<double>(),
                           h->unit_b.as<double>(), h->unit_e.as<Model>(), h->unit_f.as<int32_t>());
    else
        hipLaunchKernelGGL(kc_solver_unit<CLASSIC_FUND>, dim3((count + 63) / 64), dim3(64), SOLVE7_LDS_BYTES, s, count, h->unit_a.as<double>(),
                           h->unit_b.as<double>(), h->unit_e.as<Model>(), h->unit_f.as<int32_t>());
    HIPCHK(hipGetLastError());
    HIPCHK(hipMemcpyAsync(out, h->unit_e.p, sizeof(Model) * M * count, hipMemcpyDeviceToHost, s));
    HIPCHK(hipMemcpyAsync(n_out, h->unit_f.p, sizeof(int32_t) * count, hipMemcpyDeviceToHost, s));
    HIPCHK(hipStreamSynchronize(s));
    return MDRP_OK;
}

int mdrp_score_models(mdrp_handle *h, int kind, int mem_space, const mdrp_model *models, int num_models, const double *x1,
                      const double *x2, int n, double sq_threshold, double *scores, int32_t *counts) {
    if (!h || num_models < 0 || n < 0 || kind < 0 || kind > 5 || !scores || !counts) { g_err = "invalid argument"; return MDRP_ERR_INVALID; }
    if (num_models == 0) return MDRP_OK;
    MDRP_ENTER(h);
    hipStream_t s = h->stream;
    const int chunk = (num_models + 3) / 4;
    const size_t slots = (size_t)chunk * 4;
    int rc;
    if ((rc = h->pts.ensure(sizeof(double) * PT_STRIDE * std::max(n, 1))) || (rc = h->st.ensure(sizeof(PairState))) ||
        (rc = h->models.ensure(sizeof(Model) * slots)) || (rc = h->slot_score.ensure(sizeof(double) * slots)) ||
        (rc = h->slot_inl.ensure(sizeof(int32_t) * slots)) || (rc = h->tags[0].ensure(sizeof(uint32_t) * slots)) ||
        (rc = h->model_count[0].ensure(2 * sizeof(int32_t))))
        return rc;
    const double *x1d = x1, *x2d = x2;
    const Model *md = reinterpret_cast<const Model *>(models);
    if (mem_space == MDRP_MEM_HOST) {
        if ((rc = h->in_x1.ensure(sizeof(double) * 2 * std::max(n, 1))) || (rc = h->in_x2.ensure(sizeof(double) * 2 * std::max(n, 1)))) return rc;
        HIPCHK(hipMemcpyAsync(h->in_x1.p, x1, sizeof(double) * 2 * n, hipMemcpyHostToDevice, s));
        HIPCHK(hipMemcpyAsync(h->in_x2.p, x2, sizeof(double) * 2 * n, hipMemcpyHostToDevice, s));
        HIPCHK(hipMemcpyAsync(h->models.p, models, sizeof(Model) * num_models, hipMemcpyHostToDevice, s));
        x1d = h->in_x1.as<double>(); x2d = h->in_x2.as<double>();
        md = h->models.as<Model>();
    } else {
        HIPCHK(hipMemcpyAsync(h->models.p, models, sizeof(Model) * num_models, hipMemcpyDeviceToDevice, s));
        md = h->models.as<Model>();
    }
    if ((rc = upload_iota(s, h->tags[0].p, num_models))) return rc;
    const int32_t counts2[2] = {num_models, 0};
    HIPCHK(hipMemcpyAsync(h->model_count[0].p, counts2, 2 * sizeof(int32_t), hipMemcpyHostToDevice, s));
    if ((rc = stage_unit_pair(h, x1d, x2d, n, sq_threshold))) return rc;
    RunParams rp;
    std::memset(&rp, 0, sizeof rp);
    rp.kind = kind; rp.batch = 1; rp.n_max = std::max(n, 1); rp.chunk_len = chunk; rp.chunk_off = 0; rp.slot_stride = chunk * 4; rp.super_len = chunk;
    rp.mps = 4; rp.sample_sz = 3;
    const size_t tile_bytes = SCORE_TILE_BYTES;
    if ((rc = h->plan.ensure(sizeof(int32_t) * 8))) return rc;
    int32_t *plan = h->plan.as<int32_t>(), *totals = plan + 4;
    hipLaunchKernelGGL(k_plan, dim3(1), dim3(PLAN_THREADS), 0, s, 1, h->model_count[0].as<int32_t>(), plan, totals, SCORE_THREADS);
    const dim3 grid((unsigned)std::min(h->num_cu * 4, (num_models + SCORE_THREADS - 1) / SCORE_THREADS));
    h->ev_used = 0; h->sweep_launches = 1; h->sweep_evals = (int64_t)num_models * n;
    hipEvent_t e0, e1;
    if ((rc = get_events(h, &e0, &e1))) return rc;
    HIPCHK(hipEventRecord(e0, s));
    MDRP_SWEEP_DISPATCH(k_score, kind, grid, dim3(SCORE_THREADS), tile_bytes, s, rp, h->st.as<PairState>(), h->pts.as<double>(), md,
                        h->tags[0].as<uint32_t>(), h->model_count[0].as<int32_t>(), h->slot_score.as<double>(), h->slot_inl.as<int32_t>(), plan, totals);
    HIPCHK(hipEventRecord(e1, s));
    HIPCHK(hipGetLastError());
    const hipMemcpyKind back = mem_space == MDRP_MEM_HOST ? hipMemcpyDeviceToHost : hipMemcpyDeviceToDevice;
    HIPCHK(hipMemcpyAsync(scores, h->slot_score.p, sizeof(double) * num_models, back, s));
    HIPCHK(hipMemcpyAsync(counts, h->slot_inl.p, sizeof(int32_t) * num_models, back, s));
    return finish_timing(h);
}

int mdrp_count_candidates(mdrp_handle *h, int kind, const mdrp_model *models, int num_models, const double *x1, const double *x2,
                          int n, double sq_threshold, int32_t *candidates) {
    if (!h || num_models < 0 || n < 0 || kind < 0 || kind > 5 || !candidates || !models) { g_err = "invalid argument"; return MDRP_ERR_INVALID; }
    if (num_models == 0) return MDRP_OK;
    MDRP_ENTER(h);
    hipStream_t s = h->stream;
    const int nn = std::max(n, 1);
    const size_t slots = (size_t)num_models;
    int rc;
    if ((rc = h->pts.ensure(sizeof(double) * PT_STRIDE * nn)) || (rc = h->st.ensure(sizeof(PairState))) ||
        (rc = h->models.ensure(sizeof(Model) * slots)) || (rc = h->slot_inl.ensure(sizeof(int32_t) * slots)) ||
        (rc = h->tags[0].ensure(sizeof(uint32_t) * slots)) || (rc = h->tags_v.ensure(sizeof(uint32_t) * slots)) ||
        (rc = h->model_count[0].ensure(2 * sizeof(int32_t))) || (rc = h->surv_count.ensure(sizeof(int32_t))) ||
        (rc = h->cplan.ensure(2 * sizeof(int32_t))) || (rc = h->rfrag.ensure((size_t)((nn + 15) / 16) * 1024)) ||
        (rc = h->unit_f.ensure(sizeof(int32_t) * slots)) || (rc = h->in_x1.ensure(sizeof(double) * 2 * nn)) ||
        (rc = h->in_x2.ensure(sizeof(double) * 2 * nn)))
        return rc;
    HIPCHK(hipMemcpyAsync(h->in_x1.p, x1, sizeof(double) * 2 * n, hipMemcpyHostToDevice, s));
    HIPCHK(hipMemcpyAsync(h->in_x2.p, x2, sizeof(double) * 2 * n, hipMemcpyHostToDevice, s));
    HIPCHK(hipMemcpyAsync(h->models.p, models, sizeof(Model) * num_models, hipMemcpyHostToDevice, s));
    if ((rc = upload_iota(s, h->tags[0].p, num_models))) return rc;
    const int32_t counts2[2] = {num_models, 0};
    HIPCHK(hipMemcpyAsync(h->model_count[0].p, counts2, 2 * sizeof(int32_t), hipMemcpyHostToDevice, s));
    HIPCHK(hipMemsetAsync(h->surv_count.p, 0, sizeof(int32_t), s));
    if ((rc = stage_unit_pair(h, h->in_x1.as<double>(), h->in_x2.as<double>(), n, sq_threshold))) return rc;
    hipLaunchKernelGGL(k_frag_unit, dim3((n + 16 + 255) / 256), dim3(256), 0, s, n, h->pts.as<double>(), h->rfrag.as<uint4>());
    RunParams rp;
    std::memset(&rp, 0, sizeof rp);
    rp.kind = kind; rp.batch = 1; rp.n_max = nn; rp.slot_stride = num_models; rp.mps = 4; rp.sample_sz = 3;
    hipLaunchKernelGGL(k_count_plan, dim3(1), dim3(PLAN_THREADS), 0, s, 1, h->st.as<PairState>(), h->model_count[0].as<int32_t>(), 2, CNT_WG_MODELS, h->cplan.as<int32_t>(),
                       (int32_t *)nullptr);
    const dim3 grid((unsigned)((num_models + CNT_WG_MODELS - 1) / CNT_WG_MODELS));
    MDRP_SWEEP_DISPATCH(k_count, kind, grid, dim3(CNT_THREADS), 0, s, rp, h->st.as<PairState>(), h->rfrag.as<uint4>(), h->models.as<Model>(),
                        h->tags[0].as<uint32_t>(), h->model_count[0].as<int32_t>(), h->cplan.as<int32_t>(),
                        h->tags_v.as<uint32_t>(), h->surv_count.as<int32_t>(), (unsigned long long *)nullptr, h->unit_f.as<int32_t>());
    HIPCHK(hipGetLastError());
    HIPCHK(hipMemcpyAsync(candidates, h->unit_f.p, sizeof(int32_t) * num_models, hipMemcpyDeviceToHost, s));
    HIPCHK(hipStreamSynchronize(s));
    return MDRP_OK;
}

int mdrp_bound_models(mdrp_handle *h, int kind, const mdrp_model *models, int num_models, const double *x1, const double *x2,
                      int n, double sq_threshold, double *score_lb, int32_t *count_ub) {
    if (!h || num_models < 0 || n < 0 || kind < 0 || kind > 5 || !score_lb || !count_ub || !models) { g_err = "invalid argument"; return MDRP_ERR_INVALID; }
    if (num_models == 0) return MDRP_OK;
    MDRP_ENTER(h);
    hipStream_t s = h->stream;
    const int nn = std::max(n, 1);
    const size_t slots = (size_t)num_models;
    int rc;
    if ((rc = h->pts.ensure(sizeof(double) * PT_STRIDE * nn)) || (rc = h->st.ensure(sizeof(PairState))) ||
        (rc = h->models.ensure(sizeof(Model) * slots)) || (rc = h->slot_inl.ensure(sizeof(int32_t) * slots)) ||
        (rc = h->tags[0].ensure(sizeof(uint32_t) * slots)) || (rc = h->tags_v.ensure(sizeof(uint32_t) * slots)) ||
        (rc = h->surv_count.ensure(sizeof(int32_t))) || (rc = h->surv2_count.ensure(sizeof(int32_t))) ||
        (rc = h->cplan.ensure(2 * sizeof(int32_t))) || (rc = h->unit_a.ensure(sizeof(double) * slots)) ||
        (rc = h->unit_f.ensure(sizeof(int32_t) * slots)) || (rc = h->in_x1.ensure(sizeof(double) * 2 * nn)) ||
        (rc = h->in_x2.ensure(sizeof(double) * 2 * nn)))
        return rc;
    HIPCHK(hipMemcpyAsync(h->in_x1.p, x1, sizeof(double) * 2 * n, hipMemcpyHostToDevice, s));
    HIPCHK(hipMemcpyAsync(h->in_x2.p, x2, sizeof(double) * 2 * n, hipMemcpyHostToDevice, s));
    HIPCHK(hipMemcpyAsync(h->models.p, models, sizeof(Model) * num_models, hipMemcpyHostToDevice, s));
    if ((rc = upload_iota(s, h->tags_v.p, num_models))) return rc;
    HIPCHK(hipMemcpyAsync(h->surv_count.p, &num_models, sizeof(int32_t), hipMemcpyHostToDevice, s));
    HIPCHK(hipMemsetAsync(h->unit_a.p, 0, sizeof(double) * slots, s));
    HIPCHK(hipMemsetAsync(h->unit_f.p, 0, sizeof(int32_t) * slots, s));
    if ((rc = stage_unit_pair(h, h->in_x1.as<double>(), h->in_x2.as<double>(), n, sq_threshold))) return rc;
    RunParams rp;
    std::memset(&rp, 0, sizeof rp);
    rp.kind = kind; rp.batch = 1; rp.n_max = nn; rp.slot_stride = num_models; rp.mps = 4; rp.sample_sz = 3;
    hipLaunchKernelGGL(k_count_plan, dim3(1), dim3(PLAN_THREADS), 0, s, 1, h->st.as<PairState>(), h->surv_count.as<int32_t>(), 1, BND_THREADS,
                       h->cplan.as<int32_t>(), h->surv2_count.as<int32_t>());
    const dim3 grid((unsigned)((num_models + BND_THREADS - 1) / BND_THREADS));
    MDRP_SWEEP_DISPATCH(k_bound, kind, grid, dim3(BND_THREADS), 0, s, rp, h->st.as<PairState>(), h->pts.as<double>(), h->models.as<Model>(),
                        h->tags_v.as<uint32_t>(), h->surv_count.as<int32_t>(), h->cplan.as<int32_t>(),
                        h->tags[0].as<uint32_t>(), h->surv2_count.as<int32_t>(), (unsigned long long *)nullptr, h->unit_a.as<double>(), h->unit_f.as<int32_t>());
    HIPCHK(hipGetLastError());
    HIPCHK(hipMemcpyAsync(score_lb, h->unit_a.p, sizeof(double) * num_models, hipMemcpyDeviceToHost, s));
    HIPCHK(hipMemcpyAsync(count_ub, h->unit_f.p, sizeof(int32_t) * num_models, hipMemcpyDeviceToHost, s));
    HIPCHK(hipStreamSynchronize(s));
    return MDRP_OK;
}

int mdrp_refine_models(mdrp_handle *h, int kind, mdrp_model *models, int count, const double *x1, const double *x2,
                       const double *d1, const double *d2, int n, double scale_reproj, double weight_sampson,
                       const mdrp_bundle_opt *opt, int estimate_shift, double *final_cost) {
    if (!h || count < 0 || n < 0 || kind < 0 || kind > 5 || !opt || !models) { g_err = "invalid argument"; return MDRP_ERR_INVALID; }
    if (count == 0) return MDRP_OK;
    MDRP_ENTER(h);
    hipStream_t s = h->stream;
    int rc;
    const int nn = std::max(n, 1);
    if (kind >= MDRP_RELPOSE_5PT) {
        if ((rc = h->pts.ensure(sizeof(double) * PT_STRIDE * nn)) || (rc = h->in_x1.ensure(sizeof(double) * 2 * nn)) ||
            (rc = h->in_x2.ensure(sizeof(double) * 2 * nn)) || (rc = h->unit_e.ensure(sizeof(Model) * count)) ||
            (rc = h->unit_a.ensure(sizeof(double) * count)))
            return rc;
        HIPCHK(hipMemcpyAsync(h->in_x1.p, x1, sizeof(double) * 2 * n, hipMemcpyHostToDevice, s));
        HIPCHK(hipMemcpyAsync(h->in_x2.p, x2, sizeof(double) * 2 * n, hipMemcpyHostToDevice, s));
        HIPCHK(hipMemcpyAsync(h->unit_e.p, models, sizeof(Model) * count, hipMemcpyHostToDevice, s));
        hipLaunchKernelGGL(k_pack_unit, dim3((n + 255) / 256 + 1), dim3(256), 0, s, n, h->in_x1.as<double>(), h->in_x2.as<double>(),
                           (const double *)nullptr, (const double *)nullptr, h->pts.as<double>(), (double *)nullptr);
        MDRP_CLASSIC_LM_DISPATCH(kc_refine_unit, (count >= 2048 ? 64 : 256), kind, dim3(count), 0, s, count, h->unit_e.as<Model>(),
                                 h->pts.as<double>(), n, lm_opt(opt), h->unit_a.as<double>());
        HIPCHK(hipGetLastError());
        HIPCHK(hipMemcpyAsync(models, h->unit_e.p, sizeof(Model) * count, hipMemcpyDeviceToHost, s));
        if (final_cost) HIPCHK(hipMemcpyAsync(final_cost, h->unit_a.p, sizeof(double) * count, hipMemcpyDeviceToHost, s));
        HIPCHK(hipStreamSynchronize(s));
        return MDRP_OK;
    }
    if ((rc = h->pts.ensure(sizeof(double) * PT_STRIDE * nn)) || (rc = h->dep.ensure(sizeof(double) * 2 * nn)) ||
        (rc = h->in_x1.ensure(sizeof(double) * 2 * nn)) || (rc = h->in_x2.ensure(sizeof(double) * 2 * nn)) ||
        (rc = h->in_d1.ensure(sizeof(double) * nn)) || (rc = h->in_d2.ensure(sizeof(double) * nn)) ||
        (rc = h->unit_e.ensure(sizeof(Model) * count)) || (rc = h->unit_a.ensure(sizeof(double) * count)))
        return rc;
    HIPCHK(hipMemcpyAsync(h->in_x1.p, x1, sizeof(double) * 2 * n, hipMemcpyHostToDevice, s));
    HIPCHK(hipMemcpyAsync(h->in_x2.p, x2, sizeof(double) * 2 * n, hipMemcpyHostToDevice, s));
    HIPCHK(hipMemcpyAsync(h->in_d1.p, d1, sizeof(double) * n, hipMemcpyHostToDevice, s));
    HIPCHK(hipMemcpyAsync(h->in_d2.p, d2, sizeof(double) * n, hipMemcpyHostToDevice, s));
    HIPCHK(hipMemcpyAsync(h->unit_e.p, models, sizeof(Model) * count, hipMemcpyHostToDevice, s));
    hipLaunchKernelGGL(k_pack_unit, dim3((n + 255) / 256 + 1), dim3(256), 0, s, n, h->in_x1.as<double>(), h->in_x2.as<double>(),
                       h->in_d1.as<double>(), h->in_d2.as<double>(), h->pts.as<double>(), h->dep.as<double>());
    MDRP_LM_DISPATCH(k_refine_unit, (count >= 2048 ? 64 : 256), kind, (kind == MDRP_CALIB && estimate_shift), dim3(count), lm_list_bytes(n), s,
                     count, h->unit_e.as<Model>(), h->pts.as<double>(), h->dep.as<double>(), n, scale_reproj, weight_sampson, lm_opt(opt),
                     h->unit_a.as<double>(), lm_list_stride(n));
    HIPCHK(hipGetLastError());
    HIPCHK(hipMemcpyAsync(models, h->unit_e.p, sizeof(Model) * count, hipMemcpyDeviceToHost, s));
    if (final_cost) HIPCHK(hipMemcpyAsync(final_cost, h->unit_a.p, sizeof(double) * count, hipMemcpyDeviceToHost, s));
    HIPCHK(hipStreamSynchronize(s));
    return MDRP_OK;
}

}
```

mdrp_amd/csrc/mdrp_kernels.h:

```cpp
#pragma once
#include <hip/hip_runtime.h>
#include <float.h>
#include "mdrp_logtab.h"
#include "mdrp_math.h"

#ifdef MDRP_SECONDARY_TU
#define MDRP_GLOBAL static __global__
#else
#define MDRP_GLOBAL __global__
#endif

namespace mdrp {

constexpr int PT_STRIDE = 6;
#define MDRP_TILE_PTS 512
#define MDRP_SCORE_MINWAVES 4
constexpr int TILE_PTS = MDRP_TILE_PTS;
constexpr size_t SCORE_TILE_BYTES = (size_t)TILE_PTS * (PT_STRIDE * sizeof(double) + 4 * sizeof(float));
#define MDRP_P1F_UNROLL 8
constexpr int PRUNE_EVERY = 4;
#define MDRP_DENSE_KEY 40
#define MDRP_SOLVE_MINWAVES 2
#define MDRP_SCORE_THREADS 256
constexpr int SCORE_THREADS = MDRP_SCORE_THREADS;
// ... 1063 lines not shown
    }
    if (stats && tid == 0 && blk == 0) atomicAdd(stats, (unsigned long long)cnt * (unsigned long long)n);
}

MDRP_GLOBAL __launch_bounds__(256) void k_sort_tags(RunParams rp, const PairState *__restrict__ st, int32_t *__restrict__ model_count,
                                                   const int32_t *__restrict__ surv_count,
                                                   const uint32_t *__restrict__ tags, uint32_t *__restrict__ tags_sorted) {
    const int pair = blockIdx.x, tid = threadIdx.x;
    const PairState &ps = st[pair];
    if (!ps.active) return;
    __shared__ int s_hist[PROBE_PTS + 1], s_pos[PROBE_PTS + 1];
    __shared__ int s_dense;
    if (tid <= PROBE_PTS) s_hist[tid] = 0;
    if (tid == 0) s_dense = 0;
    __syncthreads();
    const int cnt = surv_count[pair];
    const size_t slot_base = (size_t)pair * rp.slot_stride;
    const uint32_t *src = tags + slot_base;
    uint32_t *dst = tags_sorted + slot_base;
    const int dense_min = ps.n >= 8 ? MDRP_DENSE_KEY : PROBE_PTS + 1;
    for (int i = tid; i < cnt; i += 256) atomicAdd(&s_hist[min(src[i] >> 24, (uint32_t)PROBE_PTS)], 1);
    __syncthreads();
    if (tid < 64) {
        const int v = tid < dense_min ? s_hist[tid] : 0;
        int incl = v;
#pragma unroll
        for (int o = 1; o < 64; o <<= 1) {
            const int u = __shfl_up(incl, o, 64);
            if (tid >= o) incl += u;
        }
        s_pos[tid] = incl - v;
        if (tid == 63) s_pos[64] = incl;
    }
    __syncthreads();
    const int cap = rp.slot_stride;
    for (int i = tid; i < cnt; i += 256) {
        const uint32_t t = src[i];
        const int key = (int)min(t >> 24, (uint32_t)PROBE_PTS);
        if (key >= dense_min) dst[cap - 1 - atomicAdd(&s_dense, 1)] = t & 0xFFFFFFu;
        else dst[atomicAdd(&s_pos[key], 1)] = t & 0xFFFFFFu;
    }
    __syncthreads();
    if (tid == 0) { model_count[2 * pair] = cnt - s_dense; model_count[2 * pair + 1] = s_dense; }
}

MDRP_GLOBAL __launch_bounds__(PLAN_THREADS) void k_plan(int batch, const int32_t *__restrict__ model_count, int32_t *__restrict__ plan,
                                                       int32_t *__restrict__ totals , int per_wg) {
    __shared__ int s_w[PLAN_THREADS / 64 + 1];
    int run_d = 0, run_s = 0;
    int32_t *pd = plan, *psp = plan + batch + 1;
    for (int p0 = 0; p0 < batch; p0 += PLAN_THREADS) {
        const int p = p0 + threadIdx.x;
        int bd = 0, bs = 0;
        if (p < batch) {
            bs = (model_count[2 * p] + per_wg - 1) / per_wg;
            bd = (model_count[2 * p + 1] + per_wg - 1) / per_wg;
        }
        int tot_d, tot_s;
        const int ed = plan_block_scan(bd, tot_d, s_w), es = plan_block_scan(bs, tot_s, s_w);
        if (p < batch) { pd[p] = run_d + run_s + ed + es; psp[p] = bs; }
        run_d += tot_d;
        run_s += tot_s;
    }
    if (threadIdx.x == 0) { pd[batch] = run_d + run_s; psp[batch] = 0; totals[0] = run_d; totals[1] = run_d + run_s; totals[2] = 0; }
}

template <bool POSE, bool RAWF = false>
__global__ __launch_bounds__(SCORE_THREADS, MDRP_SCORE_MINWAVES) void k_score(RunParams rp, const PairState *__restrict__ st, const double *__restrict__ pts,
                                                         const Model *__restrict__ models, const uint32_t *__restrict__ tags,
                                                         const int32_t *__restrict__ model_count, double *__restrict__ slot_score,
                                                         int32_t *__restrict__ slot_inl, const int32_t *__restrict__ plan,
                                                         int32_t *__restrict__ totals) {
    extern __shared__ double tile[];
    float4 *tile32 = reinterpret_cast<float4 *>(tile + TILE_PTS * PT_STRIDE);
    const int total = totals[1];
    const int tid = threadIdx.x;
    for (int w = blockIdx.x; w < total; w += gridDim.x) {
    const SweepItem item = sweep_item(rp, plan, model_count, tags, w, SCORE_THREADS, tid);
    const int pair = item.pair;
    const bool dense = item.dense, live = item.live;
    const PairState &ps = st[pair];
    const int n = ps.n;
    const double thr = ps.sq_thr;
    double E[9];
    float tb, Ef[9];
    const Model *mp = models + item.slot_base + item.slot;
#pragma unroll
    for (int i = 0; i < 9; ++i) E[i] = 0;
    if (live) model_matrix<POSE, RAWF>(*mp, E);
    bound_setup(E, ps, thr, Ef, tb);
    double score = 0;
    int cnt = 0;
    Prune pr(ps, live);
    const double *gp = pts + (size_t)pair * rp.n_max * PT_STRIDE;
    for (int t0 = 0; t0 < n; t0 += TILE_PTS) {
        const int npts = min(TILE_PTS, n - t0);
        __syncthreads();
        {
            const double2 *src = reinterpret_cast<const double2 *>(gp + (size_t)t0 * PT_STRIDE);
            double2 *dst = reinterpret_cast<double2 *>(tile);
            for (int i = tid; i < npts; i += SCORE_THREADS) {
                const double2 p0 = src[3 * i], p1 = src[3 * i + 1], p2 = src[3 * i + 2];
                dst[3 * i] = p0; dst[3 * i + 1] = p1; dst[3 * i + 2] = p2;
                if (!dense) store_rec32(tile32, i, p0.x, p0.y, p1.x, p1.y);
            }
        }
        __syncthreads();
        if (!pr.wave_dead) {
            if (dense) score_tile_dense<POSE>(tile, npts, E, mp, thr, score, cnt, pr);
            else score_tile_f32<POSE>(tile, tile32, npts, E, Ef, tb, mp, thr, score, cnt, pr);
        }
    }
    if (live) write_slot(slot_score, slot_inl, item.slot_base + item.slot, pr.dead, score, cnt, n, thr);
    }
}

constexpr int SCORE_WAVE_MAX_PAIRS = 128;
constexpr int SCW_THREADS = 256;
template <bool POSE, bool RAWF = false>
__global__ __launch_bounds__(SCW_THREADS) void k_score_w(RunParams rp, const PairState *__restrict__ st, const double *__restrict__ pts,
                                                         const Model *__restrict__ models, const uint32_t *__restrict__ tags ,
                                                         const int32_t *__restrict__ model_count, double *__restrict__ slot_score,
                                                         int32_t *__restrict__ slot_inl, const int32_t *__restrict__ plan ) {
    __shared__ double s_r2[SCW_THREADS / 64][64];
    const int total = plan[rp.batch];
    const int lane = threadIdx.x & 63, wave = threadIdx.x >> 6;
    const unsigned long long lt = (1ull << lane) - 1ull;
    for (int w = blockIdx.x; w < total; w += gridDim.x) {
        const int pair = plan_find(plan, rp.batch, w);
        const int i = (w - plan[pair]) * (SCW_THREADS / 64) + wave;
        const int cnt_sparse = model_count[2 * pair], cnt_dense = model_count[2 * pair + 1];
        if (i >= cnt_sparse + cnt_dense) continue;
        const PairState &ps = st[pair];
        const int n = ps.n;
        const double thr = ps.sq_thr;
        const size_t slot_base = (size_t)pair * rp.slot_stride;
        const uint32_t slot = tags[slot_base + (i < cnt_sparse ? i : rp.slot_stride - 1 - (i - cnt_sparse))];
        const Model m = models[slot_base + slot];
        double E[9], R[9], t[3] = {m.t[0], m.t[1], m.t[2]};
#pragma unroll
        for (int q = 0; q < 9; ++q) R[q] = 0;
        model_matrix<POSE, RAWF>(m, E, R);
        const Bar bar(ps);
        const double *gp = pts + (size_t)pair * rp.n_max * PT_STRIDE;
        double score = 0;
        int cnt = 0;
        bool pruned = false;
        for (int t0 = 0; t0 < n; t0 += 64) {
            const int r = t0 + lane;
            double s1 = 0;
            int c1 = 0;
            if (r < n) score_point<POSE>(gp + (size_t)r * PT_STRIDE, E, R, t, thr, s1, c1);
            const unsigned long long ball = __ballot(c1 != 0);
            if (ball) {
                if (c1) s_r2[wave][__popcll(ball & lt)] = s1;
                __builtin_amdgcn_fence(__ATOMIC_RELEASE, "wavefront");
                __builtin_amdgcn_wave_barrier();
                __builtin_amdgcn_fence(__ATOMIC_ACQUIRE, "wavefront");
                const int k = __popcll(ball);
                for (int j = 0; j < k; ++j) score += s_r2[wave][j];
                cnt += k;
                __builtin_amdgcn_wave_barrier();
            }
            const int processed = min(t0 + 64, n);
            if (bar.armed() && ((processed & 127) == 0 || processed == n) && bar.out(n, thr, processed, score, cnt)) { pruned = true; break; }
        }
        if (lane == 0) write_slot(slot_score, slot_inl, slot_base + slot, pruned, score, cnt, n, thr);
    }
}

constexpr int SPLIT_THREADS = 256;
constexpr int SPLIT_WAVES = SPLIT_THREADS / 64;
constexpr int SPLIT_HYP = 64;
constexpr int SPLIT_Q = 8;
constexpr int SPLIT_STEP = SPLIT_WAVES * SPLIT_Q;
static_assert(128 % SPLIT_STEP == 0, "the bail-out positions (every 128 records) must be step boundaries");
template <bool POSE, bool RAWF = false>
__global__ __launch_bounds__(SPLIT_THREADS, MDRP_SCORE_MINWAVES) void k_score_split(RunParams rp, const PairState *__restrict__ st, const double *__restrict__ pts,
                                                               const Model *__restrict__ models, const uint32_t *__restrict__ tags ,
                                                               const int32_t *__restrict__ model_count, double *__restrict__ slot_score,
                                                               int32_t *__restrict__ slot_inl, const int32_t *__restrict__ plan ,
                                                               const int32_t *__restrict__ totals) {
    __shared__ double s_rec[2][SPLIT_WAVES][SPLIT_Q * PT_STRIDE];
    __shared__ float4 s_rec32[2][SPLIT_WAVES][SPLIT_Q];
    __shared__ double s_r2[2][SPLIT_STEP][SPLIT_HYP];
    __shared__ int32_t s_cnt[2][SPLIT_WAVES][SPLIT_HYP];
    __shared__ unsigned long long s_dead[2];
    const int total = totals[1];
    const int lane = threadIdx.x & 63;
    const int wave = __builtin_amdgcn_readfirstlane(threadIdx.x >> 6);
    for (int w = blockIdx.x; w < total; w += gridDim.x) {
        const SweepItem item = sweep_item(rp, plan, model_count, tags, w, SPLIT_HYP, lane);
        const int pair = item.pair;
        const bool dense = item.dense, live = item.live;
        const PairState &ps = st[pair];
        const int n = ps.n;
        const double thr = ps.sq_thr;
        double E[9], R[9], t[3] = {0, 0, 0};
#pragma unroll
        for (int q = 0; q < 9; ++q) { E[q] = 0; R[q] = 0; }
        if (live) {
            const Model m = models[item.slot_base + item.slot];
            model_matrix<POSE, RAWF>(m, E, R);
            if (!RAWF) { t[0] = m.t[0]; t[1] = m.t[1]; t[2] = m.t[2]; }
        }
        float Ef[9], tb;
        bound_setup(E, ps, thr, Ef, tb);
        const Bar bar(ps);
        const double *gp = pts + (size_t)pair * rp.n_max * PT_STRIDE;
        const int steps = (n + SPLIT_STEP - 1) / SPLIT_STEP;
        double2 nx = {0, 0};
        auto fetch = [&](int j) {
            const int r = j * SPLIT_STEP + wave * SPLIT_Q + lane / 3;
            if (lane < 3 * SPLIT_Q && r < n) nx = reinterpret_cast<const double2 *>(gp + (size_t)r * PT_STRIDE)[lane % 3];
        };
        auto stage = [&](int j) {
            const int k = lane / 3, part = lane % 3;
            if (lane < 3 * SPLIT_Q && j * SPLIT_STEP + wave * SPLIT_Q + k < n) {
                reinterpret_cast<double2 *>(s_rec[j & 1][wave])[lane] = nx;
                float *q = reinterpret_cast<float *>(s_rec32[j & 1][wave]) + (k >> 1) * 8 + (k & 1);
                if (part == 0) { q[0] = (float)nx.x; q[2] = (float)nx.y; }
                else if (part == 1) { q[4] = (float)nx.x; q[6] = (float)nx.y; }
            }
        };
        fetch(0);
        stage(0);
        __syncthreads();
        double score = 0;
        int cnt = 0;
        bool dead = !live;
        bool skip = !live;
        for (int j = 0; j <= steps; ++j) {
            if (j > 0) {
                const unsigned long long dm = s_dead[(j - 1) & 1];
                if (dm == ~0ull) break;
                skip = (dm >> lane) & 1;
            }
            if (wave == 0) {
                if (j > 0) {
                    const int b = (j - 1) & 1;
                    if (!dead) {
#pragma unroll 1
                        for (int q = 0; q < SPLIT_WAVES; ++q) {
#pragma unroll
                            for (int r = 0; r < SPLIT_Q; ++r) score += s_r2[b][q * SPLIT_Q + r][lane];
                            cnt += s_cnt[b][q][lane];
                        }
                    }
                    const int processed = min(j * SPLIT_STEP, n);
                    if (bar.armed() && ((processed & 127) == 0 || processed == n)) dead = dead || bar.out(n, thr, processed, score, cnt);
                }
                if (j < steps) {
                    const unsigned long long dm = __ballot(dead);
                    if (lane == 0) s_dead[j & 1] = dm;
                }
                skip = dead;
            }
            if (j == steps) break;
            if (j + 1 < steps) fetch(j + 1);
            const int b = j & 1;
            const int valid = min(SPLIT_Q, n - (j * SPLIT_STEP + wave * SPLIT_Q));
            const double *rec = s_rec[b][wave];
            double *out = &s_r2[b][wave * SPLIT_Q][lane];
            int found = 0;
            if (dense) {
#pragma unroll 2
                for (int jj = 0; jj < SPLIT_Q; ++jj) {
                    double v = 0.0, r2;
                    if (jj < valid && !skip && record_inlier<POSE>(rec + jj * PT_STRIDE, E, R, t, thr, r2)) { v = r2; ++found; }
                    out[jj * SPLIT_HYP] = v;
                }
            } else {
#pragma unroll
                for (int jj = 0; jj < SPLIT_Q; ++jj) out[jj * SPLIT_HYP] = 0.0;
                const float4 *b32 = s_rec32[b][wave];
                f32x2 Ev[9];
#pragma unroll
                for (int q = 0; q < 9; ++q) Ev[q] = (f32x2)(Ef[q]);
                uint32_t mask = 0;
#pragma unroll
                for (int jj = 0; jj < SPLIT_Q; jj += 2) {
                    f32x2 e0, e1;
                    const f32x2 C = numerator2(Ev, b32[jj], b32[jj + 1], e0, e1);
                    mask |= (!(fabsf(C.x) > tb) ? 1u : 0u) << jj;
                    mask |= (!(fabsf(C.y) > tb) ? 1u : 0u) << (jj + 1);
                }
                mask &= valid >= SPLIT_Q ? 0xFFu : (valid > 0 ? (1u << valid) - 1u : 0u);
                if (skip) mask = 0;
                while (mask) {
                    const int jj = __ffs(mask) - 1;
                    mask &= mask - 1;
                    double r2;
                    if (record_inlier<POSE>(rec + jj * PT_STRIDE, E, R, t, thr, r2)) { out[jj * SPLIT_HYP] = r2; ++found; }
                }
            }
            s_cnt[b][wave][lane] = found;
            if (j + 1 < steps) stage(j + 1);
            __syncthreads();
        }
        if (wave == 0 && live) write_slot(slot_score, slot_inl, item.slot_base + item.slot, dead, score, cnt, n, thr);
    }
}

template <int MPS = 4, int IPL = 1>
__global__ __launch_bounds__(64) void k_scan(RunParams rp, PairState *__restrict__ st, const double *__restrict__ slot_score,
                                             const int32_t *__restrict__ slot_inl, Trigger *__restrict__ triggers,
                                             int trig_cap, const int32_t *__restrict__ model_count,
                                             unsigned long long *__restrict__ evals) {
    const int pair = blockIdx.x, lane = threadIdx.x;
    PairState &ps = st[pair];
    if (!ps.active) { if (lane == 0) ps.n_triggers = 0; return; }
    if (lane == 0 && evals) atomicAdd(evals, (unsigned long long)(model_count[2 * pair] + model_count[2 * pair + 1]) * (unsigned long long)ps.n);
    long long run_cnt = (long long)ps.best_min_cnt;
    double run_score = ps.best_min_score;
    const double nan_score = (double)ps.n * ps.sq_thr;
    int ntrig = rp.chunk_off > 0 ? ps.n_triggers : 0;
    static_assert(MPS % 4 == 0, "slots of an iteration are read as 16-byte groups");
    constexpr int NG = MPS / 4;
    const size_t slot_base = (size_t)pair * rp.slot_stride + (size_t)rp.chunk_off * MPS;
    struct Slots { int4 c[IPL][NG]; double2 s01[IPL][NG], s23[IPL][NG]; };
    auto fetch = [&](int it0) {
        Slots r;
#pragma unroll
        for (int j = 0; j < IPL; ++j) {
            const int it = it0 + IPL * lane + j;
#pragma unroll
            for (int g = 0; g < NG; ++g) {
                if (it < rp.chunk_len) {
                    r.c[j][g] = *reinterpret_cast<const int4 *>(slot_inl + slot_base + (size_t)it * MPS + 4 * g);
                    const double2 *sp = reinterpret_cast<const double2 *>(slot_score + slot_base + (size_t)it * MPS + 4 * g);
                    r.s01[j][g] = sp[0]; r.s23[j][g] = sp[1];
                } else { r.c[j][g] = make_int4(-1, -1, -1, -1); r.s01[j][g] = r.s23[j][g] = make_double2(DBL_MAX, DBL_MAX); }
            }
        }
        return r;
    };
    Slots nxt = fetch(0);
    for (int it0 = 0; it0 < rp.chunk_len; it0 += 64 * IPL) {
        const Slots cur = nxt;
        if (it0 + 64 * IPL < rp.chunk_len) nxt = fetch(it0 + 64 * IPL);
        int c[IPL][MPS];
        double s[IPL][MPS];
        long long lc = -1;
        double ls = DBL_MAX;
#pragma unroll
        for (int j = 0; j < IPL; ++j) {
#pragma unroll
            for (int g = 0; g < NG; ++g) {
                c[j][4 * g] = cur.c[j][g].x; c[j][4 * g + 1] = cur.c[j][g].y; c[j][4 * g + 2] = cur.c[j][g].z; c[j][4 * g + 3] = cur.c[j][g].w;
                s[j][4 * g] = c[j][4 * g] >= 0 ? cur.s01[j][g].x : DBL_MAX; s[j][4 * g + 1] = c[j][4 * g + 1] >= 0 ? cur.s01[j][g].y : DBL_MAX;
                s[j][4 * g + 2] = c[j][4 * g + 2] >= 0 ? cur.s23[j][g].x : DBL_MAX; s[j][4 * g + 3] = c[j][4 * g + 3] >= 0 ? cur.s23[j][g].y : DBL_MAX;
            }
            if (c[j][0] == -3) { c[j][0] = 0; s[j][0] = nan_score; }
#pragma unroll
            for (int k = 0; k < MPS; ++k) if (c[j][k] >= 0) { lc = max(lc, (long long)c[j][k]); ls = fmin(ls, s[j][k]); }
        }
        if (__all(lc <= run_cnt && !(ls < run_score))) continue;
        long long pc = lc;
        double psn = ls;
#pragma unroll
        for (int o = 1; o < 64; o <<= 1) {
            const long long vc = __shfl_up(pc, o, 64);
            const double vs = __shfl_up(psn, o, 64);
            if (lane >= o) { pc = max(pc, vc); psn = fmin(psn, vs); }
        }
        const long long tot_c = __shfl(pc, 63, 64);
        const double tot_s = __shfl(psn, 63, 64);
        long long ec = __shfl_up(pc, 1, 64);
        double es = __shfl_up(psn, 1, 64);
        if (lane == 0) { ec = -1; es = DBL_MAX; }
        long long bc = max(run_cnt, ec);
        double bs = fmin(run_score, es);
        int k_ref[IPL], k_min[IPL], cnt_min[IPL], cnt_ref[IPL], mine = 0;
        double score_min[IPL];
#pragma unroll
        for (int j = 0; j < IPL; ++j) {
            k_ref[j] = -1; k_min[j] = -1; cnt_min[j] = 0; cnt_ref[j] = 0; score_min[j] = 0;
#pragma unroll
            for (int k = 0; k < MPS; ++k) {
                if (c[j][k] >= 0) {
                    const bool more = (long long)c[j][k] > bc, better = s[j][k] < bs;
                    if (more || better) {
                        if (more) bc = c[j][k];
                        if (better) { bs = s[j][k]; k_min[j] = k; score_min[j] = s[j][k]; cnt_min[j] = c[j][k]; }
                        k_ref[j] = k; cnt_ref[j] = c[j][k];
                    }
                }
            }
            mine += k_ref[j] >= 0;
        }
        int before = mine;
#pragma unroll
        for (int o = 1; o < 64; o <<= 1) { const int v = __shfl_up(before, o, 64); if (lane >= o) before += v; }
        const int step_total = __shfl(before, 63, 64);
        int pos = ntrig + before - mine;
#pragma unroll
        for (int j = 0; j < IPL; ++j) {
            if (k_ref[j] >= 0) {
                if (pos < trig_cap) {
                    Trigger &tr = triggers[(size_t)pair * trig_cap + pos];
                    tr.iter = (uint32_t)(rp.chunk_off + it0 + IPL * lane + j); tr.k_ref = k_ref[j]; tr.k_min = k_min[j]; tr.cnt_min = cnt_min[j]; tr.score_min = score_min[j];
                    tr.ref_score = DBL_MAX; tr.ref_cnt = 0; tr.cnt_ref = cnt_ref[j];
                }
                ++pos;
            }
        }
        ntrig += step_total;
        run_cnt = max(run_cnt, tot_c);
        run_score = fmin(run_score, tot_s);
    }
    if (lane == 0) {
        ps.best_min_cnt = (uint64_t)(run_cnt < 0 ? 0 : run_cnt);
        ps.best_min_score = run_score;
        ps.n_triggers = min(ntrig, trig_cap);
    }
}

template <int KIND, bool SHIFT> struct LmTraits;
template <> struct LmTraits<0, false> { static constexpr int NP = 7; };
template <> struct LmTraits<0, true> { static constexpr int NP = 9; };
template <> struct LmTraits<1, false> { static constexpr int NP = 8; };
template <> struct LmTraits<2, false> { static constexpr int NP = 9; };

template <int KIND, bool SHIFT>
__device__ __forceinline__ constexpr int lm_col(int p) {
    return p < 7 ? p : (KIND == 0 ? p  : p + 2 );
}

struct LmOpt {
    int max_it, loss;
    double loss_scale, grad_tol, step_tol, lambda0, lambda_min, lambda_max;
    double mu = 0.5;
};

constexpr int LM_LIST_MAX_N = 8192;

__device__ __forceinline__ double uniform_f64(double x) {
    const unsigned long long b = __double_as_longlong(x);
    const unsigned lo = __builtin_amdgcn_readfirstlane((unsigned)b), hi = __builtin_amdgcn_readfirstlane((unsigned)(b >> 32));
    return __longlong_as_double(((unsigned long long)hi << 32) | lo);
}
__device__ __forceinline__ void lm_state_uniform(LmState &st) {
#pragma unroll
    for (int i = 0; i < 9; ++i) { st.R[i] = uniform_f64(st.R[i]); st.E[i] = uniform_f64(st.E[i]); st.F[i] = uniform_f64(st.F[i]); }
#pragma unroll
    for (int i = 0; i < 3; ++i) st.t[i] = uniform_f64(st.t[i]);
    st.s = uniform_f64(st.s); st.u = uniform_f64(st.u); st.v = uniform_f64(st.v);
    st.f1 = uniform_f64(st.f1); st.f2 = uniform_f64(st.f2); st.if1 = uniform_f64(st.if1); st.if2 = uniform_f64(st.if2);
}

typedef __attribute__((address_space(3))) uint16_t lds_u16;
__device__ __forceinline__ lds_u16 *lds_cast(uint16_t *p) { return (lds_u16 *)p; }

static __device__ const double g_logtab[MDRP_LOGTAB_N][2] = MDRP_LOGTAB_INIT;
__device__ __forceinline__ void lm_logtab_load(double *dst) {
    for (int i = threadIdx.x; i < 2 * MDRP_LOGTAB_N; i += blockDim.x) dst[i] = g_logtab[i >> 1][i & 1];
}

struct LmShared {
    double scratch[4 * MAX_ACC];
    int count[2][4];
    uint16_t *list;
    int stride;
    int midx;
    int mcount[4];
    const double *logtab;
    unsigned long long *stats;
    unsigned long long ev[2];
};
__device__ __forceinline__ void lm_flush_stats(LmShared &sh) {
    if (sh.stats) {
        if (sh.ev[0]) atomicAdd(sh.stats, sh.ev[0]);
        if (sh.ev[1]) atomicAdd(sh.stats + 1, sh.ev[1]);
    }
    sh.ev[0] = 0; sh.ev[1] = 0;
}

#define MDRP_LM_COST_UNROLL 1
template <int KIND>
__device__ __forceinline__ double sampson_row_weight(int loss, double lsc, double mu, double ws, double ws2, double rs) {
    return ws2 * loss_weight(loss, lsc, KIND != 0 ? ws * rs : rs, mu);
}
template <int KIND, int T, int LOSS = -1>
__device__ __forceinline__ double lm_cost(const Model &m, const double *__restrict__ pts, const double *__restrict__ dep, int n,
                          const uint8_t *__restrict__ mask, double sqrt_sr, double ws, const LmOpt &o, LmShared &sh, int buf) {
    LmState stt;
    lm_state_from_model(m, KIND != 0, stt);
    lm_state_uniform(stt);
    const int lane = threadIdx.x & 63, wave = threadIdx.x >> 6;
    const bool use_list = sh.stride > 0;
    lds_u16 *list = lds_cast(sh.list) + (size_t)buf * sh.stride;
    const int seg = ((n + T - 1) / T) * 64;
    const int lo = wave * seg;
    const lds_u16 *midx = (mask && use_list && sh.midx) ? lds_cast(sh.list) + 2 * (size_t)sh.stride : nullptr;
    const int hi = midx ? lo + sh.mcount[wave] : min(n, lo + seg);
    const int loss = LOSS >= 0 ? LOSS : o.loss;
    const double lsc = o.loss_scale, mu = o.mu, t2 = lsc * lsc;
    const double *logtab = sh.logtab;
    const bool ws_nz = ws * ws != 0.0;
    const unsigned long long lt = (1ull << lane) - 1ull;
    double cost = 0;
    int cnt = 0, evaluated = 0;
    struct Rec { double a, b, c, d, e1, e2; int id; bool ok; };
    const int last = max(n - 1, 0);
    auto fetch = [&](int base) {
        Rec r;
        const int i = base + lane;
        int ic;
        if (midx) { r.ok = i < hi; ic = r.ok ? (int)midx[i] : last; }
        else { ic = min(i, last); r.ok = (int)(i < hi) & (int)(mask ? mask[ic] != 0 : true); }
        r.id = ic;
        const double2 *P = reinterpret_cast<const double2 *>(pts + (size_t)ic * PT_STRIDE);
        const double2 p01 = P[0], p23 = P[1];
        const double2 dd = *reinterpret_cast<const double2 *>(dep + 2 * (size_t)ic);
        r.a = p01.x; r.b = p01.y; r.c = p23.x; r.d = p23.y; r.e1 = dd.x; r.e2 = dd.y;
        return r;
    };
    constexpr int U = MDRP_LM_COST_UNROLL;
    struct Trip { Rec r[U]; };
    auto fetch_trip = [&](int base) {
        Trip t;
#pragma unroll
        for (int u = 0; u < U; ++u) t.r[u] = fetch(base + 64 * u);
        return t;
    };
    auto step_trip = [&](const Trip &t, int base) {
        double vs[U], vf[U], vb[U];
        bool fwd[U], bwd[U], contrib[U];
#pragma unroll
        for (int u = 0; u < U; ++u) {
            const Rec &cur = t.r[u];
            double r[5], zf, zb;
            point_residuals<false, KIND != 0>(stt, sqrt_sr, cur.a, cur.b, cur.c, cur.d, cur.e1, cur.e2, r, zf, zb, nullptr);
            const double rs = r[0] * r[0], rf = r[1] * r[1] + r[2] * r[2], rb = r[3] * r[3] + r[4] * r[4];
            const int oki = cur.ok;
            fwd[u] = oki & (int)(zf > 0); bwd[u] = oki & (int)(zb > 0);
            const double ra = KIND != 0 ? ws * rs : rs;
            if (LOSS == 1) {
                const bool is = !(rs >= t2), ia = KIND != 0 ? !(ra >= t2) : is, jf = !(rf >= t2), jb = !(rb >= t2);
                vs[u] = ws * (is ? rs : t2); vf[u] = jf ? rf : t2; vb[u] = jb ? rb : t2;
                contrib[u] = ((oki & (int)ia & (int)ws_nz) | ((int)fwd[u] & (int)jf) | ((int)bwd[u] & (int)jb)) != 0;
            } else {
                vs[u] = ws * loss_value_tab(loss, lsc, rs, logtab); vf[u] = loss_value_tab(loss, lsc, rf, logtab); vb[u] = loss_value_tab(loss, lsc, rb, logtab);
                if (LOSS == 3 || LOSS == 4) {
                    const bool ia = LOSS == 3 || ra < t2, jf = LOSS == 3 || rf < t2, jb = LOSS == 3 || rb < t2;
                    contrib[u] = ((oki & (int)ia & (int)ws_nz) | ((int)fwd[u] & (int)jf) | ((int)bwd[u] & (int)jb)) != 0;
                } else
                    contrib[u] = ((oki & (int)(sampson_row_weight<KIND>(loss, lsc, mu, ws, ws * ws, rs) != 0.0)) | ((int)fwd[u] & (int)(loss_weight(loss, lsc, rf, mu) != 0.0)) |
                                  ((int)bwd[u] & (int)(loss_weight(loss, lsc, rb, mu) != 0.0))) != 0;
            }
        }
#pragma unroll
        for (int u = 0; u < U; ++u) {
            cost += t.r[u].ok ? vs[u] : 0.0;
            cost += fwd[u] ? vf[u] : 0.0;
            cost += bwd[u] ? vb[u] : 0.0;
            if (mask && !midx && sh.stats) evaluated += __popcll(__ballot(t.r[u].ok));
            if (use_list) {
                const unsigned long long ball = __ballot(contrib[u]);
                if (contrib[u]) list[lo + cnt + __popcll(ball & lt)] = (uint16_t)t.r[u].id;
                cnt += __popcll(ball);
            }
        }
    };
    if (!mask || midx) evaluated = max(hi - lo, 0);
    Trip A = fetch_trip(lo);
    for (int base = lo; base < hi; base += 128 * U) {
        const Trip B = fetch_trip(base + 64 * U);
        step_trip(A, base);
        A = fetch_trip(base + 128 * U);
        if (base + 64 * U < hi) step_trip(B, base + 64 * U);
    }
    if (use_list && lane == 0) sh.count[buf][wave] = cnt;
    if (sh.stats && lane == 0 && evaluated) atomicAdd(&sh.ev[0], (unsigned long long)evaluated);
    double v[1] = {cost};
    block_sum<1, T>(v, sh.scratch);
    return v[0];
}

template <int KIND, bool SHIFT, unsigned ZMASK, bool UNIT = false>
__device__ __forceinline__ void lm_accumulate_row(const double *__restrict__ Jrow, double r, double w, double *acc) {
    constexpr int NP = LmTraits<KIND, SHIFT>::NP;
    double Ja[NP];
    bool nz[NP];
#pragma unroll
    for (int q = 0; q < NP; ++q) {
        const int col = lm_col<KIND, SHIFT>(q);
        Ja[q] = Jrow[col];
        nz[q] = !((ZMASK >> col) & 1u);
        if (KIND == 1 && q == 7) { Ja[q] += Jrow[10]; nz[q] = nz[q] || !((ZMASK >> 10) & 1u); }
    }
    int idx = 0;
#pragma unroll
    for (int a = 0; a < NP; ++a) {
        const double wa = UNIT ? Ja[a] : w * Ja[a];
#pragma unroll
        for (int b = 0; b <= a; ++b, ++idx)
            if (nz[a] && nz[b]) acc[idx] += wa * Ja[b];
    }
#pragma unroll
    for (int a = 0; a < NP; ++a)
        if (nz[a]) acc[NP * (NP + 1) / 2 + a] += UNIT ? Ja[a] * r : w * Ja[a] * r;
}

template <int KIND, bool SHIFT, int LOSS = -1>
__device__ __forceinline__ void lm_accumulate_point(const LmState &stt, double2 p01, double2 p23, double2 dd,
                                                    double sqrt_sr, double ws, double ws2 , const LmOpt &o, double *acc) {
    const int loss = LOSS >= 0 ? LOSS : o.loss;
    {
        double r0, J0[LM_NPAR];
        lm_sampson_term<true, KIND != 0>(stt, p01.x, p01.y, p23.x, p23.y, r0, J0);
        const double w = sampson_row_weight<KIND>(loss, o.loss_scale, o.mu, ws, ws2, r0 * r0);
        if (w != 0.0) lm_accumulate_row<KIND, SHIFT, 0x1C0u>(J0, r0, w, acc);
    }
    {
        double r1, r2, zf, J1[LM_NPAR], J2[LM_NPAR];
        lm_forward_term<true, KIND != 0>(stt, sqrt_sr, p01.x, p01.y, p23.x, p23.y, dd.x, r1, r2, zf, J1, J2);
        const double w = !(zf > 0) ? 0.0 : loss_weight(loss, o.loss_scale, r1 * r1 + r2 * r2, o.mu);
        if (w != 0.0) {
            lm_accumulate_row<KIND, SHIFT, 0x150u, LOSS == 1>(J1, r1, w, acc);
            lm_accumulate_row<KIND, SHIFT, 0x148u, LOSS == 1>(J2, r2, w, acc);
        }
    }
    {
        double r3, r4, zb, J3[LM_NPAR], J4[LM_NPAR];
        lm_backward_term<true, KIND != 0>(stt, sqrt_sr, p01.x, p01.y, p23.x, p23.y, dd.y, r3, r4, zb, J3, J4);
        const double w = !(zb > 0) ? 0.0 : loss_weight(loss, o.loss_scale, r3 * r3 + r4 * r4, o.mu);
        if (w != 0.0) {
            lm_accumulate_row<KIND, SHIFT, 0x080u, LOSS == 1>(J3, r3, w, acc);
            lm_accumulate_row<KIND, SHIFT, 0x080u, LOSS == 1>(J4, r4, w, acc);
        }
    }
}

template <int KIND, bool SHIFT, int T, int LOSS = -1>
__device__ __forceinline__ void lm_accumulate(const Model &m, const double *__restrict__ pts, const double *__restrict__ dep, int n,
                              const uint8_t *__restrict__ mask, double sqrt_sr, double ws, double ws2, const LmOpt &o, double *acc, LmShared &sh, int buf) {
    constexpr int NP = LmTraits<KIND, SHIFT>::NP;
    constexpr int NA = NP * (NP + 1) / 2 + NP;
    LmState stt;
    lm_state_from_model(m, KIND != 0, stt);
    lm_state_uniform(stt);
#pragma unroll
    for (int i = 0; i < NA; ++i) acc[i] = 0;
    const int lane = threadIdx.x & 63, wave = threadIdx.x >> 6;
    const int seg = ((n + T - 1) / T) * 64;
    const int lo = wave * seg;
    if (sh.stride > 0) {
        const lds_u16 *list = lds_cast(sh.list) + (size_t)buf * sh.stride;
        const int cnt = sh.count[buf][wave];
        double2 n01 = make_double2(0, 0), n23 = n01, ndd = n01;
        auto fetch = [&](int k) {
            if (k < cnt) {
                const size_t i = (size_t)list[lo + k];
                const double2 *P = reinterpret_cast<const double2 *>(pts + i * PT_STRIDE);
                n01 = P[0]; n23 = P[1];
                ndd = *reinterpret_cast<const double2 *>(dep + 2 * i);
            }
        };
        fetch(lane);
        for (int k = lane; k < cnt; k += 64) {
            const double2 c01 = n01, c23 = n23, cdd = ndd;
            fetch(k + 64);
            lm_accumulate_point<KIND, SHIFT, LOSS>(stt, c01, c23, cdd, sqrt_sr, ws, ws2, o, acc);
        }
        if (sh.stats && lane == 0 && cnt) atomicAdd(&sh.ev[1], (unsigned long long)cnt);
    } else {
        const int hi = min(n, lo + seg);
        for (int i = lo + lane; i < hi; i += 64)
            if (!mask || mask[i]) {
                const double2 *P = reinterpret_cast<const double2 *>(pts + (size_t)i * PT_STRIDE);
                lm_accumulate_point<KIND, SHIFT, LOSS>(stt, P[0], P[1], *reinterpret_cast<const double2 *>(dep + 2 * (size_t)i), sqrt_sr, ws, ws2, o, acc);
            }
    }
    block_sum<NA, T>(acc, sh.scratch);
}

template <int T>
__device__ __forceinline__ void lm_mask_index(const uint8_t *__restrict__ mask, int n, LmShared &sh) {
    const int lane = threadIdx.x & 63, wave = threadIdx.x >> 6;
    const int seg = ((n + T - 1) / T) * 64;
    const int lo = wave * seg, hi = min(n, lo + seg);
    lds_u16 *midx = lds_cast(sh.list) + 2 * (size_t)sh.stride;
    const unsigned long long lt = (1ull << lane) - 1ull;
    int cnt = 0;
    for (int base = lo; base < hi; base += 64) {
        const int i = base + lane;
        const bool in = i < hi && mask[i] != 0;
        const unsigned long long ball = __ballot(in);
        if (in) midx[lo + cnt + __popcll(ball & lt)] = (uint16_t)i;
        cnt += __popcll(ball);
    }
    if (lane == 0) sh.mcount[wave] = cnt;
    __syncthreads();
}

template <int KIND, bool SHIFT, int T, int LOSS = -1>
__device__ __forceinline__ void lm_refine(Model &m, const double *__restrict__ pts, const double *__restrict__ dep, int n,
                                          const uint8_t *__restrict__ mask, double scale_reproj, double ws, const LmOpt &o_in, LmShared &sh) {
    constexpr int NP = LmTraits<KIND, SHIFT>::NP;
    constexpr int NT = NP * (NP + 1) / 2;
    const double sqrt_sr = sqrt(scale_reproj);
    const double ws2 = ws * ws;
    LmOpt o = o_in;
    o.mu = 0.5;
    int cur = 0;
    double cost = 0;
    double lambda = o.lambda0;
    bool recompute = true, first = true;
    double acc[NT + NP];
    double A[NP * NP], g[NP], sol[NP];
    Model cand = m;
    int it = 0;
    if (mask && sh.stride > 0 && sh.midx) lm_mask_index<T>(mask, n, sh);
#pragma unroll 1
    for (;;) {
        const double cost_new = lm_cost<KIND, T, LOSS>(cand, pts, dep, n, mask, sqrt_sr, ws, o, sh, first ? cur : cur ^ 1);
// ... 565 lines not shown
```

Measured before the change: 128,400.

## Defer final progress sync, merge setup memsets, cache pass sizing, add sparse list scan

Several changes land together. Host-side work per call is cut by folding the per-run memsets into one k_setup kernel, caching the pass-size decision so hipMemGetInfo is skipped on repeat calls, and deferring the final progress readback and stream sync to the next call. The scan kernel also gets a listed path: when few iterations have candidate models, it builds a bitmap of those iterations in shared memory and scans only them instead of every iteration. The changes add deferred-state bookkeeping across calls, and stats reported after a call may lag until the next call completes.

```diff
diff --git a/mdrp_amd/csrc/mdrp_capi.hip b/mdrp_amd/csrc/mdrp_capi.hip
--- a/mdrp_amd/csrc/mdrp_capi.hip
+++ b/mdrp_amd/csrc/mdrp_capi.hip
@@ -13,6 +13,7 @@
 #endif
 
 #include <algorithm>
+#include <chrono>
 #include <cmath>
 #include <cstdio>
 #include <cstdlib>
@@ -163,6 +164,8 @@
     size_t fe_n_host_cap = 0;
     DevBuf unit_a, unit_b, unit_c, unit_d, unit_e, unit_f;
     Pinned<Progress> progress_host;
+    struct Pending { bool on = false, final_done = false, lm_copied = false; int kind = 0, n_chunks = 0; uint64_t it0 = 0, super_len = 0; } pending;
+    struct OnePass { int kind = -1, batch = 0, n_max = 0, chunk_cap = 0; } one_pass;
     std::vector<std::pair<Event, Event>> ev_pool;
     std::vector<int> ev_what;
     size_t ev_used = 0;
@@ -239,6 +242,38 @@
 size_t lm_list_bytes(int n_max) { return (size_t)2 * lm_list_stride(n_max) * sizeof(uint16_t); }
 int lm_mask_index_on(int n_max) { return lm_list_stride(n_max) > 0 && (size_t)3 * lm_list_stride(n_max) * sizeof(uint16_t) <= 32768 ? 1 : 0; }
 size_t lm_final_list_bytes(int n_max) { return (size_t)(2 + lm_mask_index_on(n_max)) * lm_list_stride(n_max) * sizeof(uint16_t); }
+
+struct HostClock {
+    bool on;
+    std::chrono::steady_clock::time_point t;
+    HostClock() : on(getenv("MDRP_DEBUG") != nullptr), t(std::chrono::steady_clock::now()) {}
+    void mark(const char *what) {
+        if (!on) return;
+        const auto now = std::chrono::steady_clock::now();
+        fprintf(stderr, "[mdrp] host %-28s %8.1f us\n", what, std::chrono::duration<double, std::micro>(now - t).count());
+        t = now;
+    }
+};
+
+void account_progress(mdrp_handle *h, int kind, bool final_done, uint64_t it0, uint64_t super_len, int n_chunks) {
+    const Progress &pr = *h->progress_host;
+    h->sweep_evals += (int64_t)pr.evals;
+    h->mfma_evals += (int64_t)pr.evals_mfma;
+    h->fp64_evals += (int64_t)pr.evals_sweep;
+    h->bound_evals += (int64_t)pr.evals_bound;
+    if (final_done && pr.wish_pairs > 0)
+        h->seen_wish[kind] = (double)pr.wish_sum / (double)pr.wish_pairs;
+    if (getenv("MDRP_DEBUG"))
+        fprintf(stderr, "[mdrp] super-chunk start %llu len %llu (%d chunks): evals %llu (mfma %llu, fp32 bound %llu, fp64 sweep %llu = %.2f %%) active %d max_needed %llu\n",
+                (unsigned long long)it0, (unsigned long long)super_len, n_chunks, pr.evals, pr.evals_mfma, pr.evals_bound, pr.evals_sweep,
+                100.0 * (double)pr.evals_sweep / (double)std::max<unsigned long long>(1, pr.evals), pr.n_active, pr.max_needed);
+}
+
+void complete_pending(mdrp_handle *h) {
+    if (!h->pending.on) return;
+    h->pending.on = false;
+    account_progress(h, h->pending.kind, h->pending.final_done, h->pending.it0, h->pending.super_len, h->pending.n_chunks);
+}
 
 int get_events(mdrp_handle *h, hipEvent_t *a, hipEvent_t *b, int what = 0) {
     if (h->ev_used == h->ev_pool.size()) {
@@ -340,8 +375,9 @@
 int run_pass(mdrp_handle *h, int kind, const double *x1, const double *x2, const double *d1, const double *d2, int batch,
              int n_max, const int32_t *n_host, const mdrp_camera *cam1, const mdrp_camera *cam2, const mdrp_ransac_opt *ro,
              const mdrp_bundle_opt *bo, int chunk_cap, uint8_t *mask_dev, ResultDev *results_dev, const HostSrc *host, int batch_call,
-             const BudgetOut *bud = nullptr) {
+             const BudgetOut *bud = nullptr, bool first_pass = true, bool defer_ok = false) {
     hipStream_t s = h->stream;
+    HostClock clk;
     const int est_shift = (kind == MDRP_CALIB && ro->monodepth_estimate_shift) ? 1 : 0;
     const bool classic = kind >= MDRP_RELPOSE_5PT;
     const int mps = model_slots(kind), ssz = sample_size(kind);
@@ -357,6 +393,7 @@
     }
     const int n_tables = (int)tab_n.size();
     std::vector<uint64_t> tab_state(n_tables, ro->seed);
+    clk.mark("run_pass: group pairs");
 
     const uint64_t certain = ro->max_iterations == 0 ? 1 : std::min<uint64_t>(ro->max_iterations, ro->min_iterations + 1);
     std::vector<uint64_t> lead;
@@ -395,6 +432,13 @@
     Counters *cnt = h->counters.as<Counters>();
     const size_t groups_max = ((size_t)n_max + 15) / 16;
     const int trig_cap = chunk_cap;
+    clk.mark("run_pass: scratch");
+    const bool fuse_env = !bud && env_int("MDRP_FUSE_TAIL", ((kind == MDRP_CALIB && est_shift) || h->fuse_disabled) ? 0 : 1) != 0;
+    if (fuse_env && (rc = h->fuse.ensure(sz.fuse))) return rc;
+    hipLaunchKernelGGL(k_setup, dim3(std::min(64, (2 * batch + 16 + SETUP_THREADS - 1) / SETUP_THREADS)), dim3(SETUP_THREADS), 0, s, batch,
+                       first_pass ? h->lm_stats.as<unsigned long long>() : (unsigned long long *)nullptr, (int)(LM_STATS_BYTES / sizeof(unsigned long long)),
+                       h->counters.as<int32_t>(), (int)(sizeof(Counters) / sizeof(int32_t)), h->cand_stat.as<unsigned long long>(),
+                       h->model_count[0].as<int32_t>(), h->model_count[1].as<int32_t>(), fuse_env ? h->fuse.as<int32_t>() : (int32_t *)nullptr);
 
     {
         unsigned char *ph = h->params_host;
@@ -409,6 +453,7 @@
         HIPCHK(hipMemcpyAsync(pd, ph, sz.params, hipMemcpyHostToDevice, s));
     }
     HIPCHK(hipEventRecord(h->ev_tables, s));
+    clk.mark("run_pass: setup + upload");
 
     RunParams rp;
     std::memset(&rp, 0, sizeof rp);
@@ -438,6 +483,7 @@
     if (!host) {
         launch_prep(0, batch, s);
         HIPCHK(hipGetLastError());
+        clk.mark("run_pass: k_prep issued");
     }
     rp.inl_stat = classic ? nullptr : &cnt->progress.wish_sum;
 
@@ -449,8 +495,9 @@
     const int mask_index = lm_mask_index_on(n_max);
     const int clm_list_stride = lm_list_stride(n_max);
     const size_t clm_list_bytes = (size_t)2 * clm_list_stride * sizeof(uint16_t);
-    const bool fuse_env = !bud && env_int("MDRP_FUSE_TAIL", ((kind == MDRP_CALIB && est_shift) || h->fuse_disabled) ? 0 : 1) != 0;
     bool final_done = false;
+    const int scan_list_max = env_int("MDRP_SCAN_LIST", 1) != 0 ? std::max(0, std::min(env_int("MDRP_SCAN_LIST_MAX", SCAN_LIST_CAP), SCAN_LIST_CAP)) : 0;
+    const bool sync_each = env_int("MDRP_SYNC_EACH", 0) != 0;
     auto launch_final_of = [&](const RunParams &rf, int problems, PairState *st_f, uint8_t *mask_f, ResultDev *results_f, const int32_t *ready, int32_t *fin_done,
                                unsigned long long ticks, unsigned long long *timeouts) {
         if (classic)
@@ -488,13 +535,12 @@
         for (int c = 0; c < n_chunks; ++c) super_len += lens[c];
         if (it0 == 0) h->first_chunk = (int64_t)lens[0];
         rp.chunk_start = it0; rp.super_len = (int)super_len;
-        HIPCHK(hipMemsetAsync(h->counters.p, 0, sizeof(Counters), s));
-        if (it0 == 0) HIPCHK(hipMemsetAsync(h->cand_stat.p, 0, sizeof(unsigned long long) * 2 * batch, s));
+        const bool preset = it0 == 0;
+        if (!preset) HIPCHK(hipMemsetAsync(h->counters.p, 0, sizeof(Counters), s));
         const bool piped = n_chunks > 1 && lo_overlap;
         const bool fuse_tail = fuse_env && piped && it0 + super_len >= ro->max_iterations;
         int32_t *fz_ctl = nullptr, *fz_done = nullptr, *fz_fin = nullptr, *fz_ready = nullptr;
         if (fuse_tail) {
-            if ((rc = h->fuse.ensure(sz.fuse))) return rc;
             fz_ctl = h->fuse.as<int32_t>(); fz_done = fz_ctl + 16; fz_fin = fz_done + batch; fz_ready = fz_fin + batch;
         }
         hipStream_t aux = piped ? h->aux_stream : s, aux2 = piped ? h->aux_stream2 : s;
@@ -523,7 +569,7 @@
             uint32_t *tg = h->tags[c & 1].as<uint32_t>() + so;
             uint32_t *smp = h->samples[c & 1].as<uint32_t>();
             int32_t *mc = h->model_count[c & 1].as<int32_t>() + 2 * (size_t)p0;
-            HIPCHK(hipMemsetAsync(mc, 0, sizeof(int32_t) * 2 * pc, st_));
+            if (!(preset && c < 2)) HIPCHK(hipMemsetAsync(mc, 0, sizeof(int32_t) * 2 * pc, st_));
             if (c < 2 && presampled[c]) HIPCHK(hipStreamWaitEvent(st_, h->ev_sampled[c], 0));
             else launch_samples(st_, r.chunk_len, smp);
             hipEvent_t v0, v1;
@@ -649,7 +695,8 @@
             h->sweep_launches++;
             Trigger *trig_p = h->triggers.as<Trigger>() + (size_t)p0 * trig_cap;
             unsigned long long *scan_stats = &cnt->progress.evals_sweep;
-#define MDRP_SCAN(M, I) hipLaunchKernelGGL((k_scan<M, I>), dim3(pc), dim3(64), 0, s, r, st_p, h->slot_score.as<double>() + so, h->slot_inl.as<int32_t>() + so, trig_p, trig_cap, mcount_c, scan_stats)
+#define MDRP_SCAN(M, I) hipLaunchKernelGGL((k_scan<M, I>), dim3(pc), dim3(64), 0, s, r, st_p, h->slot_score.as<double>() + so, h->slot_inl.as<int32_t>() + so, trig_p, trig_cap, mcount_c, scan_stats, \
+                                        (const uint32_t *)tags_sc, (it0 == 0 && c == 0) ? 0 : scan_list_max)
             if (mps == 16) MDRP_SCAN(16, 1);
             else if (mps == 12) MDRP_SCAN(12, 1);
             else if (len >= 1024) MDRP_SCAN(4, 4);
@@ -715,10 +762,6 @@
             }
             int32_t *lo_plan = h->work_pair.as<int32_t>();
             hipLaunchKernelGGL(k_lo_plan, dim3(1), dim3(PLAN_THREADS), 0, s, batch, h->st.as<PairState>(), (const int32_t *)nullptr, lo_plan);
-            if (fuse_tail) {
-                HIPCHK(hipMemsetAsync(fz_ctl, 0, 64 + 2 * sizeof(int32_t) * (size_t)batch, s));
-                HIPCHK(hipMemsetAsync(fz_ready, 0xFF, sizeof(int32_t) * (size_t)batch, s));
-            }
             if (piped) { HIPCHK(hipEventRecord(h->ev_scanned[c], s)); HIPCHK(hipStreamWaitEvent(aux2, h->ev_scanned[c], 0)); }
             const int lo_blocks = h->num_cu * (lo_threads == 64 ? 8 : 2);
             const FuseTail fz = fuse_tail ? FuseTail{fz_done, fz_ready, fz_ctl, h->st.as<PairState>()} : FuseTail{nullptr, nullptr, nullptr, nullptr};
@@ -764,25 +807,28 @@
                                h->triggers.as<Trigger>(), trig_cap, &cnt->progress.n_active, &cnt->progress.max_needed,
                                (const int32_t *)nullptr, 0, 0, 0);
         HIPCHK(hipGetLastError());
+        if (it0 == 0) clk.mark("run_pass: first super-chunk issued");
+        if (defer_ok && !sync_each && ro->max_iterations == ro->min_iterations && it0 + super_len >= ro->max_iterations) {
+            h->pending.on = true; h->pending.kind = kind; h->pending.final_done = final_done; h->pending.it0 = it0; h->pending.super_len = super_len;
+            h->pending.n_chunks = n_chunks;
+            break;
+        }
         HIPCHK(hipMemcpyAsync(h->progress_host, &cnt->progress, sizeof(Progress), hipMemcpyDeviceToHost, s));
         HIPCHK(hipStreamSynchronize(s));
-        h->sweep_evals += (int64_t)h->progress_host->evals;
-        h->mfma_evals += (int64_t)h->progress_host->evals_mfma;
-        h->fp64_evals += (int64_t)h->progress_host->evals_sweep;
-        h->bound_evals += (int64_t)h->progress_host->evals_bound;
-        if (final_done && h->progress_host->wish_pairs > 0)
-            h->seen_wish[kind] = (double)h->progress_host->wish_sum / (double)h->progress_host->wish_pairs;
-        if (getenv("MDRP_DEBUG"))
-            fprintf(stderr, "[mdrp] super-chunk start %llu len %llu (%d chunks): evals %llu (mfma %llu, fp32 bound %llu, fp64 sweep %llu = %.2f %%) active %d max_needed %llu\n",
-                    (unsigned long long)it0, (unsigned long long)super_len, n_chunks, h->progress_host->evals, h->progress_host->evals_mfma,
-                    h->progress_host->evals_bound, h->progress_host->evals_sweep, 100.0 * (double)h->progress_host->evals_sweep / (double)std::max<unsigned long long>(1, h->progress_host->evals),
-                    h->progress_host->n_active, h->progress_host->max_needed);
+        account_progress(h, kind, final_done, it0, super_len, n_chunks);
         it0 += super_len;
         if (h->progress_host->n_active == 0 || it0 >= ro->max_iterations) break;
         max_needed = h->progress_host->max_needed;
     }
 
-    if (final_done) return MDRP_OK;
+    auto queue_pending = [&]() -> int {
+        if (!h->pending.on) return MDRP_OK;
+        HIPCHK(hipMemcpyAsync(h->progress_host, &cnt->progress, sizeof(Progress), hipMemcpyDeviceToHost, s));
+        HIPCHK(hipMemcpyAsync(h->lm_stats_host, h->lm_stats.p, LM_STATS_BYTES, hipMemcpyDeviceToHost, s));
+        h->pending.lm_copied = true;
+        return MDRP_OK;
+    };
+    if (final_done) return queue_pending();
     hipEvent_t f0, f1;
     if ((rc = get_events(h, &f0, &f1, 3))) return rc;
     HIPCHK(hipEventRecord(f0, s));
@@ -805,7 +851,7 @@
         h->wish_kind = kind;
     }
     HIPCHK(hipGetLastError());
-    return MDRP_OK;
+    return queue_pending();
 }
 
 int estimate_device(mdrp_handle *h, int kind, const double *x1, const double *x2, const double *d1, const double *d2, int batch,
@@ -819,14 +865,22 @@
     if (kind <= 2 && batch > 0 && n_max > 0 && (!d1 || !d2)) { g_err = "monodepth estimator needs depths"; return MDRP_ERR_INVALID; }
     if (ro->progressive_sampling) { g_err = "progressive_sampling (PROSAC, RandomSampler::initialize_prosac) is not built"; return MDRP_ERR_UNSUPPORTED; }
     if (ro->real_focal_check && (kind == MDRP_SHARED_6PT || kind == MDRP_FUNDAMENTAL_7PT)) { g_err = "real_focal_check is not built"; return MDRP_ERR_UNSUPPORTED; }
+    HostClock clk;
+    if (h->pending.on) {
+        HIPCHK(hipStreamSynchronize(h->stream));
+        complete_pending(h);
+    }
+    h->pending.lm_copied = false;
     h->last_budgets = n_budgets;
     if (h->fuse_disabled && --h->fuse_retry_in <= 0) h->fuse_disabled = false;
     h->ev_used = 0; h->sweep_ms = 0; h->sweep_launches = 0; h->sweep_evals = 0; h->mfma_evals = 0; h->fp64_evals = 0; h->bound_evals = 0; h->count_launches = 0; h->count_ms = 0; h->last_batch = batch; h->lm_cost_evals = 0; h->lm_accum_evals = 0;
     int rc;
     if ((rc = h->results.ensure(sizeof(ResultDev) * std::max(batch, 1)))) return rc;
     if ((rc = h->lm_stats.ensure(LM_STATS_BYTES))) return rc;
-    HIPCHK(hipMemsetAsync(h->lm_stats.p, 0, LM_STATS_BYTES, h->stream));
-    if (batch == 0) return MDRP_OK;
+    if (batch == 0) {
+        HIPCHK(hipMemsetAsync(h->lm_stats.p, 0, LM_STATS_BYTES, h->stream));
+        return MDRP_OK;
+    }
     std::vector<int32_t> n_host(batch);
     for (int i = 0; i < batch; ++i) {
         n_host[i] = n_per_pair ? n_per_pair[i] : n_max;
@@ -841,15 +895,25 @@
     uint64_t chunk_cap64 = std::min<uint64_t>(std::max<uint64_t>(ro->max_iterations, 1), std::max<uint64_t>(ro->min_iterations + 1, 4096));
     chunk_cap64 = std::min<uint64_t>(chunk_cap64, 16384);
     const int chunk_cap = (int)chunk_cap64;
-    size_t free_b = 0, total_b = 0;
-    HIPCHK(hipMemGetInfo(&free_b, &total_b));
-    std::vector<uint64_t> lead;
-    if (!env_chunks(lead)) lead.assign(1, 512);
-    const size_t per_pair = pass_scratch(h, kind, 2, n_max, 2, chunk_cap, lead, n_budgets).total() - pass_scratch(h, kind, 1, n_max, 1, chunk_cap, lead, n_budgets).total();
-    size_t budget = std::min<size_t>((size_t)(0.5 * (double)free_b), (size_t)96 << 30);
-    int per_pass = (int)std::max<size_t>(1, std::min<size_t>((size_t)batch, budget / per_pair));
-    per_pass = std::min(per_pass, 65535);
-    per_pass = std::max(1, std::min(per_pass, env_int("MDRP_PAIRS_PER_PASS", per_pass)));
+    clk.mark("estimate_device: checks");
+    const bool fits = !budgets && !getenv("MDRP_PAIRS_PER_PASS") && h->one_pass.kind == kind && h->one_pass.batch == batch && h->one_pass.n_max == n_max &&
+                      h->one_pass.chunk_cap == chunk_cap && batch <= 65535;
+    int per_pass = batch;
+    if (!fits) {
+        size_t free_b = 0, total_b = 0;
+        HIPCHK(hipMemGetInfo(&free_b, &total_b));
+        std::vector<uint64_t> lead;
+        if (!env_chunks(lead)) lead.assign(1, 512);
+        const size_t per_pair = pass_scratch(h, kind, 2, n_max, 2, chunk_cap, lead, n_budgets).total() - pass_scratch(h, kind, 1, n_max, 1, chunk_cap, lead, n_budgets).total();
+        size_t budget = std::min<size_t>((size_t)(0.5 * (double)free_b), (size_t)96 << 30);
+        per_pass = (int)std::max<size_t>(1, std::min<size_t>((size_t)batch, budget / per_pair));
+        per_pass = std::min(per_pass, 65535);
+        per_pass = std::max(1, std::min(per_pass, env_int("MDRP_PAIRS_PER_PASS", per_pass)));
+    }
+    h->one_pass = mdrp_handle::OnePass{};
+    if (per_pass >= batch && !budgets) h->one_pass = mdrp_handle::OnePass{kind, batch, n_max, chunk_cap};
+    clk.mark("estimate_device: pass size");
+    const bool defer_ok = per_pass >= batch && !host && !budgets;
     for (int p0 = 0; p0 < batch; p0 += per_pass) {
         const int nb = std::min(per_pass, batch - p0);
         HostSrc hs{};
@@ -859,7 +923,7 @@
         rc = run_pass(h, kind, x1 + (size_t)2 * p0 * n_max, x2 + (size_t)2 * p0 * n_max, d1 ? d1 + (size_t)p0 * n_max : nullptr,
                       d2 ? d2 + (size_t)p0 * n_max : nullptr, nb,
                       n_max, n_host.data() + p0, cam1 ? cam1 + p0 : nullptr, cam2 ? cam2 + p0 : nullptr, ro, bo, chunk_cap,
-                      mask + (size_t)p0 * n_max, h->results.as<ResultDev>() + p0, host ? &hs : nullptr, batch, budgets ? &bud : nullptr);
+                      mask + (size_t)p0 * n_max, h->results.as<ResultDev>() + p0, host ? &hs : nullptr, batch, budgets ? &bud : nullptr, p0 == 0, defer_ok);
         if (rc) return rc;
     }
     if (budgets) {
@@ -869,8 +933,11 @@
 }
 
 int finish_timing(mdrp_handle *h) {
-    if (h->lm_stats.p) HIPCHK(hipMemcpyAsync(h->lm_stats_host, h->lm_stats.p, LM_STATS_BYTES, hipMemcpyDeviceToHost, h->stream));
+    HostClock clk;
+    if (h->lm_stats.p && !h->pending.lm_copied) HIPCHK(hipMemcpyAsync(h->lm_stats_host, h->lm_stats.p, LM_STATS_BYTES, hipMemcpyDeviceToHost, h->stream));
     HIPCHK(hipStreamSynchronize(h->stream));
+    complete_pending(h);
+    clk.mark("finish_timing: synchronise");
     h->lm_cost_evals = (int64_t)h->lm_stats_host[0]; h->lm_accum_evals = (int64_t)h->lm_stats_host[1];
     h->fin_cost_evals = (int64_t)h->lm_stats_host[2]; h->fin_accum_evals = (int64_t)h->lm_stats_host[3];
     h->fuse_gate_timeouts = (int64_t)h->lm_stats_host[4]; h->fuse_wait_timeouts = (int64_t)h->lm_stats_host[5];
@@ -892,6 +959,7 @@
         h->kind_ms[k] += t; h->kind_launches[k]++;
     }
     h->sweep_ms = h->kind_ms[0]; h->count_ms = h->kind_ms[1];
+    clk.mark("finish_timing: event times");
     return MDRP_OK;
 }
 
@@ -1246,7 +1314,11 @@
 
 int mdrp_last_sweep_stats(mdrp_handle *h, double *sweep_ms, int64_t *launches, int64_t *evaluations) {
     if (!h) return MDRP_ERR_INVALID;
-    std::lock_guard<std::mutex> lock_(h->mu);
+    MDRP_ENTER(h);
+    if (h->pending.on) {
+        HIPCHK(hipStreamSynchronize(h->stream));
+        complete_pending(h);
+    }
     if (sweep_ms) *sweep_ms = h->sweep_ms;
     if (launches) *launches = h->sweep_launches;
     if (evaluations) *evaluations = h->sweep_evals;
@@ -1255,7 +1327,11 @@
 
 int mdrp_last_stats_sized(mdrp_handle *h, mdrp_stats *out, size_t out_size) {
     if (!h || !out || out_size < sizeof(double)) return MDRP_ERR_INVALID;
-    std::lock_guard<std::mutex> lock_(h->mu);
+    MDRP_ENTER(h);
+    if (h->pending.on) {
+        HIPCHK(hipStreamSynchronize(h->stream));
+        complete_pending(h);
+    }
     mdrp_stats full, *caller = out;
     out = &full;
     out->count_ms = h->count_ms; out->count_launches = h->count_launches;
diff --git a/mdrp_amd/csrc/mdrp_kernels.h b/mdrp_amd/csrc/mdrp_kernels.h
--- a/mdrp_amd/csrc/mdrp_kernels.h
+++ b/mdrp_amd/csrc/mdrp_kernels.h
@@ -1389,31 +1389,126 @@
     }
 }
 
+constexpr int SETUP_THREADS = 256;
+MDRP_GLOBAL __launch_bounds__(SETUP_THREADS) void k_setup(int batch, unsigned long long *__restrict__ lm_stats, int n_lm, int32_t *__restrict__ counters,
+                                                         int n_counters, unsigned long long *__restrict__ cand_stat, int32_t *__restrict__ mc0,
+                                                         int32_t *__restrict__ mc1, int32_t *__restrict__ fuse) {
+    const int step = gridDim.x * SETUP_THREADS, t0 = blockIdx.x * SETUP_THREADS + threadIdx.x;
+    if (lm_stats) for (int i = t0; i < n_lm; i += step) lm_stats[i] = 0ull;
+    for (int i = t0; i < n_counters; i += step) counters[i] = 0;
+    for (int i = t0; i < 2 * batch; i += step) { cand_stat[i] = 0ull; mc0[i] = 0; mc1[i] = 0; }
+    if (fuse) {
+        for (int i = t0; i < 16 + 2 * batch; i += step) fuse[i] = 0;
+        for (int i = t0; i < batch; i += step) fuse[16 + 2 * batch + i] = -1;
+    }
+}
+
+constexpr int SCAN_LIST_CAP = 1024;
+constexpr int SCAN_LIST_ITERS = 16384;
+
+template <int MPS, int IPL> struct ScanSlots { int4 c[IPL][MPS / 4]; double2 s01[IPL][MPS / 4], s23[IPL][MPS / 4]; };
+struct ScanRun { long long cnt; double score; int ntrig; };
+
+template <int MPS, int IPL>
+__device__ __forceinline__ void scan_step(const RunParams &rp, int pair, int lane, const ScanSlots<MPS, IPL> &cur, const int (&its)[IPL], double nan_score,
+                                          Trigger *__restrict__ triggers, int trig_cap, ScanRun &run) {
+    constexpr int NG = MPS / 4;
+    int c[IPL][MPS];
+    double s[IPL][MPS];
+    long long lc = -1;
+    double ls = DBL_MAX;
+#pragma unroll
+    for (int j = 0; j < IPL; ++j) {
+#pragma unroll
+        for (int g = 0; g < NG; ++g) {
+            c[j][4 * g] = cur.c[j][g].x; c[j][4 * g + 1] = cur.c[j][g].y; c[j][4 * g + 2] = cur.c[j][g].z; c[j][4 * g + 3] = cur.c[j][g].w;
+            s[j][4 * g] = c[j][4 * g] >= 0 ? cur.s01[j][g].x : DBL_MAX; s[j][4 * g + 1] = c[j][4 * g + 1] >= 0 ? cur.s01[j][g].y : DBL_MAX;
+            s[j][4 * g + 2] = c[j][4 * g + 2] >= 0 ? cur.s23[j][g].x : DBL_MAX; s[j][4 * g + 3] = c[j][4 * g + 3] >= 0 ? cur.s23[j][g].y : DBL_MAX;
+        }
+        if (c[j][0] == -3) { c[j][0] = 0; s[j][0] = nan_score; }
+#pragma unroll
+        for (int k = 0; k < MPS; ++k) if (c[j][k] >= 0) { lc = max(lc, (long long)c[j][k]); ls = fmin(ls, s[j][k]); }
+    }
+    if (__all(lc <= run.cnt && !(ls < run.score))) return;
+    long long pc = lc;
+    double psn = ls;
+#pragma unroll
+    for (int o = 1; o < 64; o <<= 1) {
+        const long long vc = __shfl_up(pc, o, 64);
+        const double vs = __shfl_up(psn, o, 64);
+        if (lane >= o) { pc = max(pc, vc); psn = fmin(psn, vs); }
+    }
+    const long long tot_c = __shfl(pc, 63, 64);
+    const double tot_s = __shfl(psn, 63, 64);
+    long long ec = __shfl_up(pc, 1, 64);
+    double es = __shfl_up(psn, 1, 64);
+    if (lane == 0) { ec = -1; es = DBL_MAX; }
+    long long bc = max(run.cnt, ec);
+    double bs = fmin(run.score, es);
+    int k_ref[IPL], k_min[IPL], cnt_min[IPL], cnt_ref[IPL], mine = 0;
+    double score_min[IPL];
+#pragma unroll
+    for (int j = 0; j < IPL; ++j) {
+        k_ref[j] = -1; k_min[j] = -1; cnt_min[j] = 0; cnt_ref[j] = 0; score_min[j] = 0;
+#pragma unroll
+        for (int k = 0; k < MPS; ++k) {
+            if (c[j][k] >= 0) {
+                const bool more = (long long)c[j][k] > bc, better = s[j][k] < bs;
+                if (more || better) {
+                    if (more) bc = c[j][k];
+                    if (better) { bs = s[j][k]; k_min[j] = k; score_min[j] = s[j][k]; cnt_min[j] = c[j][k]; }
+                    k_ref[j] = k; cnt_ref[j] = c[j][k];
+                }
+            }
+        }
+        mine += k_ref[j] >= 0;
+    }
+    int before = mine;
+#pragma unroll
+    for (int o = 1; o < 64; o <<= 1) { const int v = __shfl_up(before, o, 64); if (lane >= o) before += v; }
+    const int step_total = __shfl(before, 63, 64);
+    int pos = run.ntrig + before - mine;
+#pragma unroll
+    for (int j = 0; j < IPL; ++j) {
+        if (k_ref[j] >= 0) {
+            if (pos < trig_cap) {
+                Trigger &tr = triggers[(size_t)pair * trig_cap + pos];
+                tr.iter = (uint32_t)(rp.chunk_off + its[j]); tr.k_ref = k_ref[j]; tr.k_min = k_min[j]; tr.cnt_min = cnt_min[j]; tr.score_min = score_min[j];
+                tr.ref_score = DBL_MAX; tr.ref_cnt = 0; tr.cnt_ref = cnt_ref[j];
+            }
+            ++pos;
+        }
+    }
+    run.ntrig += step_total;
+    run.cnt = max(run.cnt, tot_c);
+    run.score = fmin(run.score, tot_s);
+}
+
 template <int MPS = 4, int IPL = 1>
 __global__ __launch_bounds__(64) void k_scan(RunParams rp, PairState *__restrict__ st, const double *__restrict__ slot_score,
                                              const int32_t *__restrict__ slot_inl, Trigger *__restrict__ triggers,
                                              int trig_cap, const int32_t *__restrict__ model_count,
-                                             unsigned long long *__restrict__ evals) {
+                                             unsigned long long *__restrict__ evals, const uint32_t *__restrict__ tags_sorted, int list_max) {
     const int pair = blockIdx.x, lane = threadIdx.x;
     PairState &ps = st[pair];
     if (!ps.active) { if (lane == 0) ps.n_triggers = 0; return; }
     if (lane == 0 && evals) atomicAdd(evals, (unsigned long long)(model_count[2 * pair] + model_count[2 * pair + 1]) * (unsigned long long)ps.n);
-    long long run_cnt = (long long)ps.best_min_cnt;
-    double run_score = ps.best_min_score;
     const double nan_score = (double)ps.n * ps.sq_thr;
-    int ntrig = rp.chunk_off > 0 ? ps.n_triggers : 0;
+    ScanRun run;
+    run.cnt = (long long)ps.best_min_cnt;
+    run.score = ps.best_min_score;
+    run.ntrig = rp.chunk_off > 0 ? ps.n_triggers : 0;
     static_assert(MPS % 4 == 0, "slots of an iteration are read as 16-byte groups");
-    constexpr int NG = MPS / 4;
     const size_t slot_base = (size_t)pair * rp.slot_stride + (size_t)rp.chunk_off * MPS;
-    struct Slots { int4 c[IPL][NG]; double2 s01[IPL][NG], s23[IPL][NG]; };
-    auto fetch = [&](int it0) {
+    typedef ScanSlots<MPS, IPL> Slots;
+    auto load = [&](auto iter_of) {
         Slots r;
 #pragma unroll
         for (int j = 0; j < IPL; ++j) {
-            const int it = it0 + IPL * lane + j;
-#pragma unroll
-            for (int g = 0; g < NG; ++g) {
-                if (it < rp.chunk_len) {
+            const int it = iter_of(j);
+#pragma unroll
+            for (int g = 0; g < MPS / 4; ++g) {
+                if (it >= 0 && it < rp.chunk_len) {
                     r.c[j][g] = *reinterpret_cast<const int4 *>(slot_inl + slot_base + (size_t)it * MPS + 4 * g);
                     const double2 *sp = reinterpret_cast<const double2 *>(slot_score + slot_base + (size_t)it * MPS + 4 * g);
                     r.s01[j][g] = sp[0]; r.s23[j][g] = sp[1];
@@ -1422,84 +1517,73 @@
         }
         return r;
     };
-    Slots nxt = fetch(0);
-    for (int it0 = 0; it0 < rp.chunk_len; it0 += 64 * IPL) {
-        const Slots cur = nxt;
-        if (it0 + 64 * IPL < rp.chunk_len) nxt = fetch(it0 + 64 * IPL);
-        int c[IPL][MPS];
-        double s[IPL][MPS];
-        long long lc = -1;
-        double ls = DBL_MAX;
-#pragma unroll
-        for (int j = 0; j < IPL; ++j) {
-#pragma unroll
-            for (int g = 0; g < NG; ++g) {
-                c[j][4 * g] = cur.c[j][g].x; c[j][4 * g + 1] = cur.c[j][g].y; c[j][4 * g + 2] = cur.c[j][g].z; c[j][4 * g + 3] = cur.c[j][g].w;
-                s[j][4 * g] = c[j][4 * g] >= 0 ? cur.s01[j][g].x : DBL_MAX; s[j][4 * g + 1] = c[j][4 * g + 1] >= 0 ? cur.s01[j][g].y : DBL_MAX;
-                s[j][4 * g + 2] = c[j][4 * g + 2] >= 0 ? cur.s23[j][g].x : DBL_MAX; s[j][4 * g + 3] = c[j][4 * g + 3] >= 0 ? cur.s23[j][g].y : DBL_MAX;
-            }
-            if (c[j][0] == -3) { c[j][0] = 0; s[j][0] = nan_score; }
-#pragma unroll
-            for (int k = 0; k < MPS; ++k) if (c[j][k] >= 0) { lc = max(lc, (long long)c[j][k]); ls = fmin(ls, s[j][k]); }
-        }
-        if (__all(lc <= run_cnt && !(ls < run_score))) continue;
-        long long pc = lc;
-        double psn = ls;
-#pragma unroll
-        for (int o = 1; o < 64; o <<= 1) {
-            const long long vc = __shfl_up(pc, o, 64);
-            const double vs = __shfl_up(psn, o, 64);
-            if (lane >= o) { pc = max(pc, vc); psn = fmin(psn, vs); }
-        }
-        const long long tot_c = __shfl(pc, 63, 64);
-        const double tot_s = __shfl(psn, 63, 64);
-        long long ec = __shfl_up(pc, 1, 64);
-        double es = __shfl_up(psn, 1, 64);
-        if (lane == 0) { ec = -1; es = DBL_MAX; }
-        long long bc = max(run_cnt, ec);
-        double bs = fmin(run_score, es);
-        int k_ref[IPL], k_min[IPL], cnt_min[IPL], cnt_ref[IPL], mine = 0;
-        double score_min[IPL];
-#pragma unroll
-        for (int j = 0; j < IPL; ++j) {
-            k_ref[j] = -1; k_min[j] = -1; cnt_min[j] = 0; cnt_ref[j] = 0; score_min[j] = 0;
-#pragma unroll
-            for (int k = 0; k < MPS; ++k) {
-                if (c[j][k] >= 0) {
-                    const bool more = (long long)c[j][k] > bc, better = s[j][k] < bs;
-                    if (more || better) {
-                        if (more) bc = c[j][k];
-                        if (better) { bs = s[j][k]; k_min[j] = k; score_min[j] = s[j][k]; cnt_min[j] = c[j][k]; }
-                        k_ref[j] = k; cnt_ref[j] = c[j][k];
-                    }
+    bool listed = false;
+    if constexpr (MPS == 4) {
+        const int n_sparse = model_count[2 * pair], n_dense = model_count[2 * pair + 1], n_list = n_sparse + n_dense;
+        listed = tags_sorted != nullptr && list_max > 0 && n_sparse >= 0 && n_dense >= 0 && n_list <= min(min(list_max, SCAN_LIST_CAP), rp.slot_stride) &&
+                 rp.chunk_len <= SCAN_LIST_ITERS && run.score <= nan_score;
+        if (listed) {
+            constexpr int WORDS = SCAN_LIST_ITERS / 32, WPL = WORDS / 64;
+            __shared__ uint32_t s_bits[WORDS];
+            __shared__ int32_t s_iters[SCAN_LIST_CAP];
+#pragma unroll
+            for (int w = 0; w < WPL; ++w) s_bits[WPL * lane + w] = 0;
+            __syncthreads();
+            const uint32_t *tl = tags_sorted + (size_t)pair * rp.slot_stride;
+            for (int i = lane; i < n_list; i += 64) {
+                const uint32_t tag = tl[i < n_sparse ? i : rp.slot_stride - 1 - (i - n_sparse)] & 0xFFFFFFu;
+                const int it = (int)(tag >> 2) - rp.chunk_off;
+                if (it >= 0 && it < rp.chunk_len) atomicOr(&s_bits[it >> 5], 1u << (it & 31));
+            }
+            __syncthreads();
+            uint32_t wv[WPL];
+            int mine = 0;
+#pragma unroll
+            for (int w = 0; w < WPL; ++w) { wv[w] = s_bits[WPL * lane + w]; mine += __popc(wv[w]); }
+            int incl = mine;
+#pragma unroll
+            for (int o = 1; o < 64; o <<= 1) { const int v = __shfl_up(incl, o, 64); if (lane >= o) incl += v; }
+            const int n_iters = __shfl(incl, 63, 64);
+            int at = incl - mine;
+#pragma unroll
+            for (int w = 0; w < WPL; ++w) {
+                uint32_t m = wv[w];
+                while (m) {
+                    const int b = __ffs(m) - 1;
+                    m &= m - 1;
+                    if (at < SCAN_LIST_CAP) s_iters[at] = (WPL * lane + w) * 32 + b;
+                    ++at;
                 }
             }
-            mine += k_ref[j] >= 0;
-        }
-        int before = mine;
-#pragma unroll
-        for (int o = 1; o < 64; o <<= 1) { const int v = __shfl_up(before, o, 64); if (lane >= o) before += v; }
-        const int step_total = __shfl(before, 63, 64);
-        int pos = ntrig + before - mine;
-#pragma unroll
-        for (int j = 0; j < IPL; ++j) {
-            if (k_ref[j] >= 0) {
-                if (pos < trig_cap) {
-                    Trigger &tr = triggers[(size_t)pair * trig_cap + pos];
-                    tr.iter = (uint32_t)(rp.chunk_off + it0 + IPL * lane + j); tr.k_ref = k_ref[j]; tr.k_min = k_min[j]; tr.cnt_min = cnt_min[j]; tr.score_min = score_min[j];
-                    tr.ref_score = DBL_MAX; tr.ref_cnt = 0; tr.cnt_ref = cnt_ref[j];
+            __syncthreads();
+            for (int e0 = 0; e0 < n_iters; e0 += 64 * IPL) {
+                int its[IPL];
+#pragma unroll
+                for (int j = 0; j < IPL; ++j) {
+                    const int e = e0 + IPL * lane + j;
+                    its[j] = e < n_iters ? s_iters[e] : -1;
                 }
-                ++pos;
-            }
-        }
-        ntrig += step_total;
-        run_cnt = max(run_cnt, tot_c);
-        run_score = fmin(run_score, tot_s);
+                const Slots cur = load([&](int j) { return its[j]; });
+                scan_step<MPS, IPL>(rp, pair, lane, cur, its, nan_score, triggers, trig_cap, run);
+            }
+        }
+    }
+    if (!listed) {
+        auto fetch = [&](int it0) { return load([&](int j) { return it0 + IPL * lane + j; }); };
+        Slots nxt = fetch(0);
+        for (int it0 = 0; it0 < rp.chunk_len; it0 += 64 * IPL) {
+            const Slots cur = nxt;
+            if (it0 + 64 * IPL < rp.chunk_len) nxt = fetch(it0 + 64 * IPL);
+            int its[IPL];
+#pragma unroll
+            for (int j = 0; j < IPL; ++j) its[j] = it0 + IPL * lane + j;
+            scan_step<MPS, IPL>(rp, pair, lane, cur, its, nan_score, triggers, trig_cap, run);
+        }
     }
     if (lane == 0) {
-        ps.best_min_cnt = (uint64_t)(run_cnt < 0 ? 0 : run_cnt);
-        ps.best_min_score = run_score;
-        ps.n_triggers = min(ntrig, trig_cap);
+        ps.best_min_cnt = (uint64_t)(run.cnt < 0 ? 0 : run.cnt);
+        ps.best_min_score = run.score;
+        ps.n_triggers = min(run.ntrig, trig_cap);
     }
 }
 
```

After: 128,200. Within noise of the previous version (-0.2%).
